# world-modelz/world-modelz

Hardware: AMD Instinct MI355X
Metric: denoise-step latent-frames/sec (forward, 32x16x16 latent clips) (higher is better)
Workload: dtype bf16; 1 GPU; BASELINE.json configs[3] per GPU: VqVideoDiffusionModel.forward, B=8 clips/GPU of 32x16x16 latents, codebook 1024, dim 256, dim_head 128, heads 1, extents 3,3,3, depth 4, mlp 256; clips_per_gpu=8, codebook=1024, parallelism=clips sharded over 1 rank(s), no data-path collective

## Files before the change

### world_modelz_amd/csrc/fused_common.h

```cpp
#pragma once
#include "wmz_common.h"
#include <stdlib.h>

#define WMZ_FENCE()                        \
  do {                                     \
    asm volatile("" ::: "memory");         \
    __builtin_amdgcn_sched_barrier(0);     \
  } while (0)

namespace {

constexpr int TW = 32;
#ifndef WMZ_FUSED_FW
#define WMZ_FUSED_FW 8
#endif
constexpr int FW = WMZ_FUSED_FW;
constexpr int NTHR = FW * 64;
constexpr int HALF = 16384;
constexpr int PIECES = HALF / 1024;
#ifndef WMZ_FUSED_HPS
#define WMZ_FUSED_HPS 2
#endif
constexpr int HPS = WMZ_FUSED_HPS;
constexpr int SLAB = HPS * HALF;
#ifndef WMZ_FUSED_RING
#define WMZ_FUSED_RING (WMZ_FUSED_HPS == 1 ? 4 : 2)
#endif
constexpr int RING = WMZ_FUSED_RING;
constexpr int WPP = SLAB / 1024 / FW;
constexpr int VECB = 8192;
constexpr int MC = 32;

struct WStream {
  int dbg;
  const char* src;
  char* ring;
  int issue_slot;
  int cur;
  int half;
  int wave;
  int probe;
  long long* ts;
  int tot, t1, t2, t3;
  int all;
};

__device__ __forceinline__ void ws_issue(WStream& ws) {
  ws.t1 = ws.t2; ws.t2 = ws.t3; ws.t3 = ws.tot;
  ws.all += WPP;
  if (ws.dbg & 2) return;
  char* dst = ws.ring + ws.issue_slot * SLAB;
#pragma unroll
  for (int i = 0; i < WPP; ++i)
    __builtin_amdgcn_global_load_lds((const __attribute__((address_space(1))) void*)(ws.src + i * 1024),
                                     (__attribute__((address_space(3))) void*)(dst + i * 1024), 16, 0, 0);
  ws.src += SLAB;
  ws.issue_slot = ws.issue_slot == RING - 1 ? 0 : ws.issue_slot + 1;
}

__device__ __forceinline__ void ws_wait(WStream& ws) {
  constexpr int YB = WPP * (RING - 2);
  static_assert(YB == 4 || YB == 0, "literals below");
  const int e = ws.tot - (RING == 4 ? ws.t1 : (RING == 3 ? ws.t2 : ws.t3));
  if (!(ws.dbg & 2)) {
#define WMZ_VMC(n) case n: if (YB == 4) asm volatile("s_waitcnt vmcnt(" #n " + 4)" ::: "memory"); else asm volatile("s_waitcnt vmcnt(" #n ")" ::: "memory"); break;
    switch (e) {
      WMZ_VMC(0) WMZ_VMC(1) WMZ_VMC(2) WMZ_VMC(3) WMZ_VMC(4) WMZ_VMC(5) WMZ_VMC(6) WMZ_VMC(7) WMZ_VMC(8) WMZ_VMC(9)
      WMZ_VMC(10) WMZ_VMC(11) WMZ_VMC(12) WMZ_VMC(13) WMZ_VMC(14) WMZ_VMC(15) WMZ_VMC(16) WMZ_VMC(17) WMZ_VMC(18)
      WMZ_VMC(19) WMZ_VMC(20) WMZ_VMC(21) WMZ_VMC(22) WMZ_VMC(23) WMZ_VMC(24) WMZ_VMC(25) WMZ_VMC(26) WMZ_VMC(27)
      WMZ_VMC(28) WMZ_VMC(29) WMZ_VMC(30) WMZ_VMC(31) WMZ_VMC(32)
      default: asm volatile("s_waitcnt vmcnt(32)" ::: "memory"); break;
    }
#undef WMZ_VMC
  }
  if (ws.probe && ws.ts) ws.ts[ws.probe] = __builtin_readcyclecounter();
  if (!(ws.dbg & 4)) __builtin_amdgcn_s_barrier();
  if (ws.probe && ws.ts) ws.ts[ws.probe + 1] = __builtin_readcyclecounter();
}
__device__ __forceinline__ void ws_release(WStream& ws) { ws.cur = ws.cur == RING - 1 ? 0 : ws.cur + 1; }
__device__ __forceinline__ void ws_extra(WStream& ws, int n) { ws.tot += n; ws.all += n; }
__device__ __forceinline__ void vm_wait(int n) {
#define WMZ_VMW(k) case k: asm volatile("s_waitcnt vmcnt(" #k ")" ::: "memory"); break;
  switch (n) {
    WMZ_VMW(0) WMZ_VMW(1) WMZ_VMW(2) WMZ_VMW(3) WMZ_VMW(4) WMZ_VMW(5) WMZ_VMW(6) WMZ_VMW(7) WMZ_VMW(8) WMZ_VMW(9) WMZ_VMW(10)
    WMZ_VMW(11) WMZ_VMW(12) WMZ_VMW(13) WMZ_VMW(14) WMZ_VMW(15) WMZ_VMW(16) WMZ_VMW(17) WMZ_VMW(18) WMZ_VMW(19) WMZ_VMW(20)
    WMZ_VMW(21) WMZ_VMW(22) WMZ_VMW(23) WMZ_VMW(24) WMZ_VMW(25) WMZ_VMW(26) WMZ_VMW(27) WMZ_VMW(28) WMZ_VMW(29) WMZ_VMW(30)
    WMZ_VMW(31) WMZ_VMW(32) WMZ_VMW(33) WMZ_VMW(34) WMZ_VMW(35) WMZ_VMW(36) WMZ_VMW(37) WMZ_VMW(38) WMZ_VMW(39) WMZ_VMW(40)
    WMZ_VMW(41) WMZ_VMW(42) WMZ_VMW(43) WMZ_VMW(44) WMZ_VMW(45) WMZ_VMW(46) WMZ_VMW(47)
    default: asm volatile("s_waitcnt vmcnt(48)" ::: "memory"); break;
  }
#undef WMZ_VMW
}
__device__ __forceinline__ void vm_wait_since(const WStream& ws, int mark) { vm_wait(ws.all - mark); }

struct NoSide { static constexpr int kValuPerMfma = 0; __device__ __forceinline__ void operator()(int) const {} };
template <int VPM, typename F> struct SideWork {
  static constexpr int kValuPerMfma = VPM;
  F f;
  __device__ __forceinline__ void operator()(int g) const { f(g); }
};
template <int VPM, typename F> __device__ __forceinline__ SideWork<VPM, F> side_work(F f) { return SideWork<VPM, F>{f}; }

template <int NB, int KS, typename BGet, typename Side = NoSide>
__device__ __forceinline__ void gemm_stage_b(f32x16 (&acc)[NB], BGet bget, const char* ring0, WStream& ws, int lane,
                                             Side side = Side()) {
  constexpr int NP = NB * KS;
  static_assert(NP % PIECES == 0, "a stage is a whole number of slabs");
  constexpr int AG = 4, GPS = PIECES / AG;
  Frag8<bf16_t> bcur, bnext = bget(0);
  bcur = bnext;
#pragma unroll
  for (int sl = 0; sl < NP / PIECES; ++sl) {
    if (ws.half == 0) ws_wait(ws);
    const char* slab = ring0 + ws.cur * SLAB + ws.half * HALF + lane * 16;
    Frag8<bf16_t> af[2][AG];
    if (!(ws.dbg & 1)) {
#pragma unroll
      for (int j = 0; j < AG; ++j) af[0][j].v = *reinterpret_cast<const s16x8*>(slab + j * 1024);
    }
    if (ws.half == 0) ws_issue(ws);
    if (ws.probe && ws.ts) ws.ts[ws.probe + 2] = __builtin_readcyclecounter();
    if (!(ws.dbg & 1)) {
#pragma unroll
      for (int gq = 0; gq < GPS; ++gq) {
        if (gq == 1 && ws.probe && ws.ts) { asm volatile("s_waitcnt lgkmcnt(0)" ::: "memory"); ws.ts[ws.probe + 3] = __builtin_readcyclecounter(); }
        if (gq + 1 < GPS) {
#pragma unroll
          for (int j = 0; j < AG; ++j)
            af[(gq + 1) & 1][j].v = *reinterpret_cast<const s16x8*>(slab + ((gq + 1) * AG + j) * 1024);
        }
#pragma unroll
        for (int j = 0; j < AG; ++j) {
          const int idx = sl * PIECES + gq * AG + j;
          if (idx % NB == 0) {
            bcur = bnext;
            if (idx / NB + 1 < KS) bnext = bget(idx / NB + 1);
          }
          mma32(acc[idx % NB], af[gq & 1][j], bcur);
        }
        side(sl * GPS + gq);
        if (gq + 1 < GPS) __builtin_amdgcn_sched_group_barrier(0x100, AG, 0);
        if constexpr (Side::kValuPerMfma > 0) {
#pragma unroll
          for (int j = 0; j < AG; ++j) {
            __builtin_amdgcn_sched_group_barrier(0x008, 1, 0);
            __builtin_amdgcn_sched_group_barrier(0x002, Side::kValuPerMfma, 0);
          }
        } else {
          __builtin_amdgcn_sched_group_barrier(0x008, AG, 0);
        }
        WMZ_FENCE();
      }
    }
    if (ws.half == HPS - 1) { ws_release(ws); ws.half = 0; }
    else ++ws.half;
  }
}
template <int NB, int KS, typename Side = NoSide>
__device__ __forceinline__ void gemm_stage(f32x16 (&acc)[NB], const Frag8<bf16_t> (&bop)[KS], const char* ring0, WStream& ws,
                                           int lane, Side side = Side()) {
  gemm_stage_b<NB, KS>(acc, [&](int s) { return bop[s]; }, ring0, ws, lane, side);
}

__device__ __forceinline__ f32x16 lds_vec16(const float* p) {
  const f32x4 a = *reinterpret_cast<const f32x4*>(p), b = *reinterpret_cast<const f32x4*>(p + 4);
  const f32x4 c = *reinterpret_cast<const f32x4*>(p + 8), d = *reinterpret_cast<const f32x4*>(p + 12);
  f32x16 v;
#pragma unroll
  for (int i = 0; i < 4; ++i) { v[i] = a[i]; v[4 + i] = b[i]; v[8 + i] = c[i]; v[12 + i] = d[i]; }
  return v;
}
template <int NB>
__device__ __forceinline__ void add_vec(f32x16 (&acc)[NB], const float* vec ) {
#pragma unroll
  for (int b = 0; b < NB; ++b) acc[b] += lds_vec16(vec + 16 * b);
}
template <int NB>
__device__ __forceinline__ void init_vec(f32x16 (&acc)[NB], const float* vec) {
#pragma unroll
  for (int b = 0; b < NB; ++b) acc[b] = lds_vec16(vec + 16 * b);
}

__device__ __forceinline__ void pack8(Frag8<bf16_t>& f, const float (&y)[8]) {
#ifdef WMZ_OP16_F16
  const s16x4 lo = cvt_pk4_bf16(y[0], y[1], y[2], y[3]), hi = cvt_pk4_bf16(y[4], y[5], y[6], y[7]);
  s16x8 v = __builtin_shufflevector(lo, hi, 0, 1, 2, 3, 4, 5, 6, 7);
#else
  s16x8 v;
#pragma unroll
  for (int j = 0; j < 8; ++j) v[j] = (short)f32_to_bf16_bits(y[j]);
#endif
  asm volatile("" : "+v"(v));
  f.v = v;
}

template <int KS>
__device__ __forceinline__ void load_bop(Frag8<bf16_t> (&bop)[KS], const bf16_t* half_row) {
#pragma unroll
  for (int s = 0; s < KS; ++s) bop[s].v = *reinterpret_cast<const s16x8*>(half_row + 8 * s);
}

__device__ __forceinline__ s16x8 gload_untracked(const bf16_t* p) {
  s16x8 v;
  asm volatile("global_load_dwordx4 %0, %1, off" : "=v"(v) : "v"(p) : "memory");
  return v;
}
template <int KS>
__device__ __forceinline__ void wait_untracked(Frag8<bf16_t> (&b)[KS]) {
  if (WPP * (RING - 1) == 6) asm volatile("s_waitcnt vmcnt(6)" ::: "memory");
  else asm volatile("s_waitcnt vmcnt(4)" ::: "memory");
#pragma unroll
  for (int s = 0; s < KS; ++s) asm volatile("" : "+v"(b[s].v));
}
__device__ __forceinline__ void vec_dma(float* vecs, const float* src, int wave, int lane) {
#pragma unroll
  for (int i = 0; i < 8 / FW; ++i) {
    const int kb = wave * (8 / FW) + i;
    __builtin_amdgcn_global_load_lds((const __attribute__((address_space(1))) void*)(src + kb * 256 + lane * 4),
                                     (__attribute__((address_space(3))) void*)(reinterpret_cast<char*>(vecs) + kb * 1024), 16, 0, 0);
  }
}
template <int NB>
__device__ __forceinline__ void add_bop(f32x16 (&acc)[NB], const Frag8<bf16_t> (&bop)[2 * NB]) {
#pragma unroll
  for (int b = 0; b < NB; ++b)
#pragma unroll
    for (int i = 0; i < 16; ++i) acc[b][i] = op16_add_to(acc[b][i], (unsigned short)bop[2 * b + (i >> 3)].v[i & 7]);
}

template <int KS>
__device__ __forceinline__ void load_bop_tiled(Frag8<bf16_t> (&bop)[KS], const bf16_t* tile, int lane) {
#pragma unroll
  for (int s = 0; s < KS; ++s) bop[s].v = *reinterpret_cast<const s16x8*>(tile + (s * 64 + lane) * 8);
}
template <int KS>
__device__ __forceinline__ void store_bop_tiled(bf16_t* tile, const Frag8<bf16_t> (&bop)[KS], int lane, HalfGuard& hg) {
  if (hg.on()) {
#pragma unroll
    for (int s = 0; s < KS; ++s) hg.see(bop[s].v);
    hg.fold(WMZ_HG_STREAM);
  }
#pragma unroll
  for (int s = 0; s < KS; ++s) *reinterpret_cast<s16x8*>(tile + (s * 64 + lane) * 8) = bop[s].v;
}

__device__ __forceinline__ void stage_dma128(char* stg, const bf16_t* src, int rowf, long tok0, int ntok, int lane) {
#pragma unroll
  for (int p = 0; p < 8; ++p) {
    const int r = p * 4 + (lane >> 4), pc = lane & 15;
    const long row = tok0 + r < ntok ? tok0 + r : ntok - 1;
    __builtin_amdgcn_global_load_lds((const __attribute__((address_space(1))) void*)(src + row * rowf + ((pc ^ (r & 15)) << 3)),
                                     (__attribute__((address_space(3))) void*)(stg + p * 1024), 16, 0, 0);
  }
}
__device__ __forceinline__ Frag8<bf16_t> stage_get(const char* stg, int t, int c) {
  Frag8<bf16_t> f;
  f.v = *reinterpret_cast<const s16x8*>(stg + t * 256 + ((c ^ (t & 15)) << 4));
  return f;
}
__device__ __forceinline__ void stage_put(char* stg, const s16x8& v, int t, int c) {
  *reinterpret_cast<s16x8*>(stg + t * 256 + ((c ^ (t & 15)) << 4)) = v;
}
template <int ROWF>
__device__ __forceinline__ void stage_flush(const char* stg, bf16_t* dst, long tok0, int ntok, int col0, int lane, HalfGuard& hg,
                                            unsigned kind) {
  asm volatile("" : "+s"(tok0), "+v"(lane));
  s16x8 v[8];
#pragma unroll
  for (int p = 0; p < 8; ++p) v[p] = *reinterpret_cast<const s16x8*>(stg + p * 1024 + lane * 16);
  if (hg.on()) {
#pragma unroll
    for (int p = 0; p < 8; ++p) hg.see(v[p]);
    hg.fold(kind);
  }
#pragma unroll
  for (int p = 0; p < 8; ++p) {
    const int r = p * 4 + (lane >> 4), pc = lane & 15;
    const int c = pc ^ (r & 15);
    if (tok0 + r < ntok) *reinterpret_cast<s16x8*>(dst + (tok0 + r) * ROWF + col0 + c * 8) = v[p];
  }
}
template <int ROWF>
__device__ __forceinline__ void stage_flush(const char* stg, bf16_t* dst, long tok0, int ntok, int col0, int lane) {
  HalfGuard none;
  stage_flush<ROWF>(stg, dst, tok0, ntok, col0, lane, none, 0u);
}
__device__ __forceinline__ void frag_park(char* stg, int slot, const Frag8<bf16_t>& f, int lane) {
  *reinterpret_cast<s16x8*>(stg + slot * 1024 + lane * 16) = f.v;
}
__device__ __forceinline__ Frag8<bf16_t> frag_unpark(const char* stg, int slot, int lane) {
  Frag8<bf16_t> f;
  f.v = *reinterpret_cast<const s16x8*>(stg + slot * 1024 + lane * 16);
  return f;
}

__device__ __forceinline__ void store_tile128(char* stg, bf16_t* dst, int rowf, long tok0, int ntok, int col0,
                                              const Frag8<bf16_t> (&b)[8], int lane, HalfGuard& hg) {
  const int t = lane & 31, h = lane >> 5;
#pragma unroll
  for (int s = 0; s < 8; ++s) stage_put(stg, b[s].v, t, h * 8 + s);
  if (rowf == 128) stage_flush<128>(stg, dst, tok0, ntok, col0, lane, hg, WMZ_HG_QKV);
  else stage_flush<256>(stg, dst, tok0, ntok, col0, lane, hg, WMZ_HG_QKV);
}
__device__ __forceinline__ void store_tile128(char* stg, bf16_t* dst, int rowf, long tok0, int ntok, int col0,
                                              const Frag8<bf16_t> (&b)[8], int lane) {
  HalfGuard none;
  store_tile128(stg, dst, rowf, tok0, ntok, col0, b, lane, none);
}
__device__ __forceinline__ void store_tile256(char* stg, bf16_t* dst, long tok0, int ntok, const Frag8<bf16_t> (&b)[16],
                                              int lane, HalfGuard& hg) {
  const int t = lane & 31, h = lane >> 5;
#pragma unroll
  for (int hh = 0; hh < 2; ++hh) {
    if (h == hh) {
#pragma unroll
      for (int s = 0; s < 16; ++s) stage_put(stg, b[s].v, t, s);
    }
    stage_flush<256>(stg, dst, tok0, ntok, hh * 128, lane, hg, WMZ_HG_STREAM);
  }
}
__device__ __forceinline__ void store_tile256(char* stg, bf16_t* dst, long tok0, int ntok, const Frag8<bf16_t> (&b)[16],
                                              int lane) {
  HalfGuard none;
  store_tile256(stg, dst, tok0, ntok, b, lane, none);
}

template <int NB>
__device__ __forceinline__ void acc_from_bop(f32x16 (&acc)[NB], const Frag8<bf16_t> (&bop)[2 * NB]) {
#pragma unroll
  for (int b = 0; b < NB; ++b)
#pragma unroll
    for (int i = 0; i < 16; ++i) acc[b][i] = bf16_bits_to_f32((unsigned short)bop[2 * b + (i >> 3)].v[i & 7]);
#ifdef WMZ_OP16_F16
#pragma unroll
  for (int b = 0; b < NB; ++b) asm volatile("" : "+v"(acc[b]));
#endif
}
template <int NB>
__device__ __forceinline__ void bop_from_acc(Frag8<bf16_t> (&bop)[2 * NB], const f32x16 (&acc)[NB]) {
#pragma unroll
  for (int b = 0; b < NB; ++b)
#pragma unroll
    for (int m = 0; m < 2; ++m) {
      float y[8];
#pragma unroll
      for (int j = 0; j < 8; ++j) y[j] = acc[b][8 * m + j];
      pack8(bop[2 * b + m], y);
    }
}

template <int NB>
__device__ __forceinline__ void ln_stats(const f32x16 (&acc)[NB], float eps, float& rstd, float& mr) {
  constexpr int NF = NB * 32;
  f32x16 sv = acc[0];
#pragma unroll
  for (int b = 1; b < NB; ++b) sv += acc[b];
  float s = 0.f;
#pragma unroll
  for (int i = 0; i < 16; ++i) s += sv[i];
  s = wave_halves_sum(s);
  const float mean = s / (float)NF;
  f32x16 qv = (f32x16)(0.f);
#pragma unroll
  for (int b = 0; b < NB; ++b) { const f32x16 d = acc[b] - mean; qv += d * d; }
  float q = 0.f;
#pragma unroll
  for (int i = 0; i < 16; ++i) q += qv[i];
  q = wave_halves_sum(q);
  rstd = rsqrtf(q / (float)NF + eps);
  mr = -mean * rstd;
}
__device__ __forceinline__ void ln_block(Frag8<bf16_t>& lo, Frag8<bf16_t>& hi, const f32x16& x, float rstd, float mr) {
  const f32x16 y = x * rstd + mr;
  float a[8], b[8];
#pragma unroll
  for (int j = 0; j < 8; ++j) { a[j] = y[j]; b[j] = y[8 + j]; }
  pack8(lo, a);
  pack8(hi, b);
}
__device__ __forceinline__ void put_stats(float* st, long tok, int ntok, float rstd, float mr, int lane) {
  if (lane < 32 && tok < ntok) {
    st[tok] = -mr / rstd;
    st[(long)ntok + tok] = rstd;
  }
}
template <int NB>
__device__ __forceinline__ void ln_to_bop(Frag8<bf16_t> (&bop)[2 * NB], const f32x16 (&acc)[NB], float eps, float* st = nullptr,
                                          long tok = 0, int ntok = 0, int lane = 0) {
  float rstd, mr;
  ln_stats<NB>(acc, eps, rstd, mr);
  if (st != nullptr) put_stats(st, tok, ntok, rstd, mr, lane);
#pragma unroll
  for (int b = 0; b < NB; ++b) ln_block(bop[2 * b], bop[2 * b + 1], acc[b], rstd, mr);
}
template <int NB>
__device__ __forceinline__ void ln_and_pack(Frag8<bf16_t> (&lnb)[2 * NB], Frag8<bf16_t> (&xb)[2 * NB], const f32x16 (&acc)[NB],
                                            float eps, float* st = nullptr, long tok = 0, int ntok = 0, int lane = 0) {
  float rstd, mr;
  ln_stats<NB>(acc, eps, rstd, mr);
  if (st != nullptr) put_stats(st, tok, ntok, rstd, mr, lane);
#pragma unroll
  for (int b = 0; b < NB; ++b) {
    ln_block(lnb[2 * b], lnb[2 * b + 1], acc[b], rstd, mr);
    float a[8], c[8];
#pragma unroll
    for (int j = 0; j < 8; ++j) { a[j] = acc[b][j]; c[j] = acc[b][8 + j]; }
    pack8(xb[2 * b], a);
    pack8(xb[2 * b + 1], c);
  }
}

template <int N> __device__ __forceinline__ void zero_acc(f32x16 (&acc)[N]) {
#pragma unroll
  for (int b = 0; b < N; ++b) acc[b] = (f32x16)(0.f);
}
}
```

### world_modelz_amd/csrc/layer_fused.hip

```cpp
#include "fused_common.h"
#include "fused_pack_rows.h"
#include "wmz_debug.h"

namespace {

struct FusedParams {
  const bf16_t* o;
  const bf16_t* x;
  bf16_t* xo;
  bf16_t* q;
  bf16_t* kv;
  const char* wpack;
  const float* vec;
  int ntok;
  float eps;
  const int64_t* z; const float *emb, *pos_s, *pos_h, *pos_w; int S, H, W, num_classes;
  int dbg;
  int rows_out, rows_in, row0;
  int xflags;
  bf16_t* x1o; bf16_t* xo_rm; int kv_combined;
  float* st_ff; float* st_attn;
  bf16_t* zt;
  long long* ts;
};
#define WMZ_TS(slot)                                                                                      \
  do {                                                                                                    \
    if (P.ts != nullptr && blockIdx.x == 0 && lane == 0) P.ts[wave * 64 + (slot)] = __builtin_readcyclecounter(); \
  } while (0)
__device__ __forceinline__ long src_row(const FusedParams& P, long t) {
  if (P.rows_out == 0) return t;
  const int c = (int)t / P.rows_out;
  return (long)c * P.rows_in + P.row0 + ((int)t - c * P.rows_out);
}

template <int F>
__device__ __forceinline__ void embed_bop(Frag8<bf16_t> (&bop)[F / 16], const FusedParams& P, long t, bool ok, int h) {
  (void)ok;
  const long ts = src_row(P, t);
  const int w = (int)(ts % P.W), hh = (int)((ts / P.W) % P.H), s = (int)((ts / ((long)P.W * P.H)) % P.S);
  long tk = P.z[ts];
  tk = tk < 0 ? 0 : (tk >= P.num_classes ? P.num_classes - 1 : tk);
  const float* e = P.emb + tk * F + h * (F / 2);
  const float* a = P.pos_s + (long)s * F + h * (F / 2);
  const float* b = P.pos_h + (long)hh * F + h * (F / 2);
  const float* d = P.pos_w + (long)w * F + h * (F / 2);
#pragma unroll
  for (int c = 0; c < F / 16; ++c) {
    float y[8];
#pragma unroll
    for (int q = 0; q < 2; ++q) {
      const f32x4 ev = *reinterpret_cast<const f32x4*>(e + 8 * c + 4 * q);
      const f32x4 av = *reinterpret_cast<const f32x4*>(a + 8 * c + 4 * q);
      const f32x4 bv = *reinterpret_cast<const f32x4*>(b + 8 * c + 4 * q);
      const f32x4 dv = *reinterpret_cast<const f32x4*>(d + 8 * c + 4 * q);
      const f32x4 yv = ev + ((av + bv) + dv);
#pragma unroll
      for (int r = 0; r < 4; ++r) y[4 * q + r] = yv[r];
    }
    pack8(bop[c], y);
    if ((c & 1) == 1) WMZ_FENCE();
  }
}

template <int F>
__device__ __forceinline__ void embed_coop(Frag8<bf16_t> (&bop)[F / 16], char* stg, const FusedParams& P, long tok0, int lane) {
  static_assert(F == 256, "one 1 KB fp32 row per wave instruction");
  const long last = P.ntok - 1;
  const long ts0 = src_row(P, tok0 < last ? tok0 : last);
  const int h0 = (int)((ts0 / 16) % P.H), s = (int)((ts0 / (16L * P.H)) % P.S);
  const int h1 = h0 + 1 < P.H ? h0 + 1 : h0;
  const f32x4 ps = *reinterpret_cast<const f32x4*>(P.pos_s + (long)s * F + lane * 4);
  const f32x4 a0 = ps + *reinterpret_cast<const f32x4*>(P.pos_h + (long)h0 * F + lane * 4);
  const f32x4 a1 = ps + *reinterpret_cast<const f32x4*>(P.pos_h + (long)h1 * F + lane * 4);
  f32x4 pw[16];
#pragma unroll
  for (int w = 0; w < 16; ++w) pw[w] = *reinterpret_cast<const f32x4*>(P.pos_w + (long)w * F + lane * 4);
  const int t = lane & 31, hl = lane >> 5;
  int tkv;
  {
    const long tt = tok0 + t < last ? tok0 + t : last;
    long tk = P.z[ts0 + (tt - (tok0 < last ? tok0 : last))];
    tk = tk < 0 ? 0 : (tk >= P.num_classes ? P.num_classes - 1 : tk);
    tkv = (int)tk;
  }
#pragma unroll
  for (int p = 0; p < 2; ++p) {
    const f32x4 a = p ? a1 : a0;
#pragma unroll
    for (int i = 0; i < 16; ++i) {
      const long tk = __builtin_amdgcn_readlane(tkv, 16 * p + i);
      const f32x4 e = *reinterpret_cast<const f32x4*>(P.emb + tk * F + lane * 4);
      const f32x4 y = e + (a + pw[i]);
      s16x4 pk;
#pragma unroll
      for (int r = 0; r < 4; ++r) pk[r] = (short)f32_to_bf16_bits(y[r]);
      *reinterpret_cast<s16x4*>(stg + i * 512 + ((((lane >> 1) ^ i) << 4) | ((lane & 1) << 3))) = pk;
    }
    if ((t >> 4) == p) {
      const int tl = t & 15;
#pragma unroll
      for (int c = 0; c < F / 16; ++c)
        bop[c].v = *reinterpret_cast<const s16x8*>(stg + tl * 512 + (((hl * 16 + c) ^ tl) << 4));
    }
  }
}

__device__ __forceinline__ void store_z_tiled(bf16_t* zt, long tok0, int c, const f32x16& z, int lane) {
#pragma unroll
  for (int j = 0; j < 2; ++j) {
    float y[8];
#pragma unroll
    for (int i = 0; i < 8; ++i) y[i] = z[8 * j + i];
    Frag8<bf16_t> f;
    pack8(f, y);
    *reinterpret_cast<s16x8*>(zt + tok0 * 256 + ((2 * c + j) * 64 + lane) * 8) = f.v;
  }
}

template <int D, int I, int M, bool HEAD, bool TAIL>
__global__ __launch_bounds__(NTHR, 8 / FW) void layer_fused_kernel(FusedParams P) {
  static_assert(D == 256 && M == 256 && I == 128, "built for the default denoiser widths");
  extern __shared__ __attribute__((aligned(16))) char smem[];
  const int tid = threadIdx.x, lane = tid & 63;
  const int wave = __builtin_amdgcn_readfirstlane(tid >> 6);
  const int h = lane >> 5;
  float* vecs = reinterpret_cast<float*>(smem);
  const char* ring0 = smem + VECB;
  HalfGuard hg;
  WStream ws;
  ws.ring = smem + VECB + wave * (SLAB / FW);
  ws.src = P.wpack + wave * (SLAB / FW) + lane * 16;
  ws.half = 0;
  ws.issue_slot = 0;
  ws.cur = 0;
  ws.dbg = P.dbg;
  ws.tot = ws.t1 = ws.t2 = ws.t3 = 0;
  ws.all = 0;
  ws.wave = wave;
  ws.probe = 0;
  ws.ts = (P.ts != nullptr && blockIdx.x == 0 && lane == 0) ? P.ts + wave * 64 : nullptr;
  WMZ_TS(0);
  const long tok0 = (long)blockIdx.x * (TW * FW) + wave * TW;
  const long tok = tok0 + (lane & 31);
  const long tokc = tok < P.ntok ? tok : P.ntok - 1;
  const bool tile_ok = tok0 < P.ntok;
  const long tok0c = tile_ok ? tok0 : (P.ntok >= 32 ? P.ntok - 32 : 0);
  char* stg = smem + VECB + RING * SLAB + wave * 8192;
  static_assert(VECB == 8192 && 8 % FW == 0, "vector block is 2048 floats, 8 / FW KB per wave");
  const float* v_bout = vecs + h * (D / 2);
  const float* v_b1 = vecs + D + h * (MC / 2);
  const float* v_b2 = vecs + D + M + h * (D / 2);
  const float* v_bk = vecs + 2 * D + M + h * (I / 2);
  const float* v_bv = v_bk + I;

  Frag8<bf16_t> qkvb[I / 16];
  f32x16 xr[D / 32];
  Frag8<bf16_t> xb[D / 16];
  if constexpr (HEAD) {
    stage_dma128(stg, P.o, I, tok0, P.ntok, lane);
    vec_dma(vecs, P.vec, wave, lane);
#pragma unroll
    for (int i = 0; i < RING - 1; ++i) ws_issue(ws);
    const bool xt = (P.xflags & WMZ_FUSED_X_IN_TILED) != 0;
    {
      const bf16_t* xp = xt ? P.x + src_row(P, tok0c) * D + lane * 8 : P.x + src_row(P, tokc) * D + h * (D / 2);
      const int xs = xt ? 64 * 8 : 8;
#pragma unroll
      for (int s = 0; s < D / 16; ++s) xb[s].v = gload_untracked(xp + s * xs);
    }
    ws_extra(ws, D / 16);
    WMZ_TS(1);
    if (WPP * (RING - 1) == 6) asm volatile("s_waitcnt vmcnt(22)" ::: "memory");
    else asm volatile("s_waitcnt vmcnt(20)" ::: "memory");
    static_assert(WPP * (RING - 1) == 6 || WPP * (RING - 1) == 4, "literals above");
    __builtin_amdgcn_s_barrier();
    WMZ_TS(44);
    init_vec<D / 32>(xr, v_bout);
    WMZ_TS(2);
    {
      const int t = lane & 31;
      gemm_stage_b<D / 32, I / 16>(xr, [&](int ks) { return stage_get(stg, t, h * (I / 16) + ks); }, ring0, ws, lane);
    }
    wait_untracked<D / 16>(xb);
    WMZ_TS(45);
    add_bop<D / 32>(xr, xb);
    const bool x1_hat = (P.xflags & WMZ_FUSED_X1_NORMALISED) != 0;
    if (P.x1o != nullptr && !x1_hat) {
      bop_from_acc<D / 32>(xb, xr);
      store_tile256(stg, P.x1o, tok0, P.ntok, xb, lane, hg);
      ws_extra(ws, 16);
    }
    WMZ_TS(3);
    ln_to_bop<D / 32>(xb, xr, P.eps, P.st_ff, tok, P.ntok, lane);
    if (P.st_ff != nullptr) ws_extra(ws, 2);
    if (P.x1o != nullptr && x1_hat) {
      store_tile256(stg, P.x1o, tok0, P.ntok, xb, lane, hg);
      ws_extra(ws, 16);
    }
    WMZ_TS(4);
#pragma unroll
    for (int sx = 8; sx < 16; ++sx) frag_park(stg, sx - 8, xb[sx], lane);
    {
      auto lnb = [&](int sx) { return sx < 8 ? xb[sx] : frag_unpark(stg, sx - 8, lane); };
      auto gelu_n = [&](float (&y)[8], const f32x16& zz, int first, int yo, int n) {
#pragma unroll
        for (int j = 0; j < 4; ++j) if (j < n) y[yo + j] = wmz_gelu_fast(zz[first + j]);
      };
      f32x16 zc[1], zn[1];
      Frag8<bf16_t> gb[2], gn[2];
      float y[8];
      init_vec<1>(zc, v_b1);
      gemm_stage_b<1, D / 16>(zc, lnb, ring0, ws, lane);
      const bool zsave = P.zt != nullptr && tile_ok;
      if (zsave) { store_z_tiled(P.zt, tok0, 0, zc[0], lane); ws_extra(ws, 2); }
      WMZ_TS(5);
      init_vec<1>(zn, v_b1 + MC);
      gemm_stage_b<1, D / 16>(zn, lnb, ring0, ws, lane, side_work<9>([&](int g) {
        gelu_n(y, zc[0], 4 * g, (g & 1) * 4, 4);
        if (g & 1) pack8(gb[g >> 1], y);
      }));
      if (zsave) { store_z_tiled(P.zt, tok0, 1, zn[0], lane); ws_extra(ws, 2); }
      zc[0] = zn[0];
      WMZ_TS(6);
#pragma unroll 1
      for (int c = 1; c < M / MC - 1; ++c) {
        if (c == 4) ws.probe = 48;
        gemm_stage<D / 32, MC / 16>(xr, gb, ring0, ws, lane, side_work<5>([&](int g) {
          gelu_n(y, zc[0], 2 * g, 2 * g, 2);
          if (g == 3) pack8(gn[0], y);
        }));
        ws.probe = 0;
        WMZ_TS(5 + 3 * c);
        init_vec<1>(zn, v_b1 + (c + 1) * MC);
        if (c == 4) ws.probe = 52;
        gemm_stage_b<1, D / 16>(zn, lnb, ring0, ws, lane, side_work<5>([&](int g) {
          gelu_n(y, zc[0], 8 + 2 * g, 2 * g, 2);
          if (g == 3) pack8(gn[1], y);
        }));
        ws.probe = 0;
        if (zsave) { store_z_tiled(P.zt, tok0, c + 1, zn[0], lane); ws_extra(ws, 2); }
        WMZ_TS(7 + 3 * c);
        zc[0] = zn[0];
        gb[0] = gn[0];
        gb[1] = gn[1];
      }
      gemm_stage<D / 32, MC / 16>(xr, gb, ring0, ws, lane, side_work<9>([&](int g) {
        gelu_n(y, zc[0], 4 * g, (g & 1) * 4, 4);
        if (g & 1) pack8(gn[g >> 1], y);
      }));
      gemm_stage<D / 32, MC / 16>(xr, gn, ring0, ws, lane);
      WMZ_TS(29);
    }
    add_vec<D / 32>(xr, v_b2);
    Frag8<bf16_t> x2b[D / 16];
    if constexpr (TAIL) {
      ln_and_pack<D / 32>(xb, x2b, xr, P.eps, P.st_attn, tok, P.ntok, lane);
      if (P.st_attn != nullptr) ws_extra(ws, 2);
    }
    else bop_from_acc<D / 32>(x2b, xr);
    WMZ_TS(30);
    if (P.xflags & WMZ_FUSED_X_OUT_TILED) { if (tile_ok) store_bop_tiled<D / 16>(P.xo + tok0 * D, x2b, lane, hg); }
    else store_tile256(stg, P.xo, tok0, P.ntok, x2b, lane, hg);
    ws_extra(ws, 16);
    if (P.xo_rm != nullptr) {
      if (TAIL && (P.xflags & WMZ_FUSED_XRM_NORMALISED)) store_tile256(stg, P.xo_rm, tok0, P.ntok, xb, lane, hg);
      else store_tile256(stg, P.xo_rm, tok0, P.ntok, x2b, lane, hg);
      ws_extra(ws, 16);
    }
    WMZ_TS(31);
    if constexpr (TAIL) {
      f32x16 qa[I / 32];
      zero_acc(qa);
      gemm_stage<I / 32, D / 16>(qa, x2b, ring0, ws, lane);
      WMZ_TS(32);
      bop_from_acc<I / 32>(qkvb, qa);
    }
  } else {
    if (P.z != nullptr) {
      const bool coop = P.W == 16 && (P.H * 16) % 32 == 0 && (P.rows_out == 0 || (P.rows_out % 32 == 0 && P.rows_in % 32 == 0 && P.row0 % 32 == 0));
      if (coop) embed_coop<D>(xb, stg, P, tok0, lane);
      else embed_bop<D>(xb, P, tokc, true, h);
    }
    else if (P.xflags & WMZ_FUSED_X_IN_TILED) load_bop_tiled<D / 16>(xb, P.x + src_row(P, tok0c) * D, lane);
    else load_bop<D / 16>(xb, P.x + src_row(P, tokc) * D + h * (D / 2));
    f32x4 vecv[8 / FW];
#pragma unroll
    for (int i = 0; i < 8 / FW; ++i) vecv[i] = *reinterpret_cast<const f32x4*>(P.vec + (tid + i * NTHR) * 4);
#pragma unroll
    for (int i = 0; i < RING - 1; ++i) ws_issue(ws);
#pragma unroll
    for (int i = 0; i < 8 / FW; ++i) *reinterpret_cast<f32x4*>(vecs + (tid + i * NTHR) * 4) = vecv[i];
    __syncthreads();
    if (P.z != nullptr) {
      if (P.xflags & WMZ_FUSED_X_OUT_TILED) { if (tile_ok) store_bop_tiled<D / 16>(P.xo + tok0 * D, xb, lane, hg); }
      else store_tile256(stg, P.xo, tok0, P.ntok, xb, lane, hg);
      ws_extra(ws, 16);
      if (P.xo_rm != nullptr && !(P.xflags & WMZ_FUSED_XRM_NORMALISED)) { store_tile256(stg, P.xo_rm, tok0, P.ntok, xb, lane, hg); ws_extra(ws, 16); }
    }
    {
      f32x16 qa[I / 32];
      zero_acc(qa);
      gemm_stage<I / 32, D / 16>(qa, xb, ring0, ws, lane);
      bop_from_acc<I / 32>(qkvb, qa);
    }
    acc_from_bop<D / 32>(xr, xb);
    ln_to_bop<D / 32>(xb, xr, P.eps, P.st_attn, tok, P.ntok, lane);
    if (P.st_attn != nullptr) ws_extra(ws, 2);
    if (P.xo_rm != nullptr && (P.xflags & WMZ_FUSED_XRM_NORMALISED)) { store_tile256(stg, P.xo_rm, tok0, P.ntok, xb, lane, hg); ws_extra(ws, 16); }
  }
  if constexpr (TAIL) {
    f32x16 ka[I / 32];
    Frag8<bf16_t> kb[I / 16];
    init_vec<I / 32>(ka, v_bk);
    store_tile128(stg, P.q, I, tok0, P.ntok, 0, qkvb, lane, hg);
    ws_extra(ws, 8);
    WMZ_TS(33);
    gemm_stage<I / 32, D / 16>(ka, xb, ring0, ws, lane);
    WMZ_TS(34);
    bop_from_acc<I / 32>(kb, ka);
    if (P.kv_combined) store_tile128(stg, P.kv, 2 * I, tok0, P.ntok, 0, kb, lane, hg);
    else store_tile128(stg, P.kv, I, tok0, P.ntok, 0, kb, lane, hg);
    ws_extra(ws, 8);
    init_vec<I / 32>(ka, v_bv);
    WMZ_TS(35);
    gemm_stage<I / 32, D / 16>(ka, xb, ring0, ws, lane);
    WMZ_TS(36);
    bop_from_acc<I / 32>(kb, ka);
    if (P.kv_combined) store_tile128(stg, P.kv, 2 * I, tok0, P.ntok, I, kb, lane, hg);
    else store_tile128(stg, P.kv + (long)P.ntok * I, I, tok0, P.ntok, 0, kb, lane, hg);
  }
  asm volatile("s_waitcnt vmcnt(0)" ::: "memory");
  hg.commit();
  WMZ_TS(37);
}

}

static int fused_launch(FusedParams& P, int ntok, int D, int I, int M, int has_head, int has_tail, void* stream);
static FusedParams fused_params(const void* o, const void* x, void* x_out, void* q_out, void* kv_out, const void* wpack,
                                const float* vec, int ntok, float eps) {
  FusedParams P = {};
  P.o = (const bf16_t*)o; P.x = (const bf16_t*)x; P.xo = (bf16_t*)x_out; P.q = (bf16_t*)q_out; P.kv = (bf16_t*)kv_out;
  P.wpack = (const char*)wpack; P.vec = vec; P.ntok = ntok; P.eps = eps;
  return P;
}
static long long* g_fused_ts = nullptr;
static int g_fused_dbg = 0;
#ifndef WMZ_OP16_F16
extern "C" int wmz_debug_fused_knobs(int dbg) { g_fused_dbg = dbg; return WMZ_OK; }
extern "C" int wmz_debug_fused_timestamps(void* buf) { g_fused_ts = (long long*)buf; return WMZ_OK; }
#endif

extern "C" int WMZ_FN(wmz_layer_fused_fwd)(const void* o, const void* x, void* x_out, void* q_out, void* kv_out,
                                   const void* wpack, const float* vec, int ntok, int D, int I, int M, int has_head,
                                   int has_tail, float eps, void* stream) {
  return WMZ_FN(wmz_layer_fused_fwd_planes)(o, x, x_out, q_out, kv_out, wpack, vec, 1, 1, 1, ntok, D, I, M, has_head, has_tail, 0,
                                    eps, stream);
}

namespace {
struct PackRows { FusedPackRow row[24]; int n; long total8, padded8; };
struct VecJobG { const float *bout, *b1, *w1, *be2, *b2, *wk, *wv, *be1, *bv; float* vec; };
static_assert(sizeof(VecJobG) == 80, "table layouts are part of the C ABI");

__device__ __forceinline__ void pack_group(const FusedPackRow& B, long g) {
  const long e = g * 8;
  const int NB = (int)B.N / 32;
  const int piece = (int)(e / 512), lane = (int)((e % 512) / 8);
  const int s = piece / NB, b = piece % NB;
  const int r = lane & 31, h = lane >> 5;
  const int bpg = (int)B.gn / 32, spg = (int)B.gk / 16;
  const int f = (b / bpg) * (int)B.gn + ((r >> 2) & 1) * ((int)B.gn / 2) + (b % bpg) * 16 + (r & 3) + 4 * (r >> 3);
  const int k0 = (s / spg) * (int)B.gk + h * ((int)B.gk / 2) + (s % spg) * 8;
  const float rg = B.rgamma ? B.rgamma[f] : 1.f;
  s16x8 v;
#pragma unroll
  for (int j = 0; j < 8; ++j) {
    float x = B.w[(long)f * B.rs + (long)(k0 + j) * B.ks] * rg;
    if (B.gamma) x *= B.gamma[k0 + j];
    v[j] = (short)f32_to_bf16_bits(x);
  }
  *reinterpret_cast<s16x8*>(B.dst + e) = v;
}
__global__ __launch_bounds__(256) void fused_pack_kernel(PackRows P) {
  const long g8 = (long)blockIdx.x * 256 + threadIdx.x;
  if (g8 < P.total8) {
    int bi = 0;
#pragma unroll 1
    for (int i = 1; i < P.n; ++i) if (g8 >= P.row[i].start8) bi = i;
    const FusedPackRow& B = P.row[bi];
    pack_group(B, g8 - B.start8);
  } else if (g8 < P.padded8) {
    *reinterpret_cast<s16x8*>(P.row[0].dst + g8 * 8) = (s16x8)(0);
  }
}
__global__ __launch_bounds__(256) void fused_pack_table_kernel(const FusedPackRow* __restrict__ rows, int nblk, long total8) {
  const long g8 = (long)blockIdx.x * 256 + threadIdx.x;
  if (g8 >= total8) return;
  int lo = 0, hi = nblk - 1;
  while (lo < hi) {
    const int mid = (lo + hi + 1) >> 1;
    if (rows[mid].start8 <= g8) lo = mid; else hi = mid - 1;
  }
  const FusedPackRow B = rows[lo];
  pack_group(B, g8 - B.start8);
}

__device__ __forceinline__ void pack_vec_entry(const VecJobG& P, int t, int lane, int D, int I, int M) {
  const float* row = nullptr; const float* vecb = nullptr; float base = 0.f;
  if (t < D) base = P.bout ? P.bout[t] : 0.f;
  else if (t < D + M) { if (P.b1) { base = P.b1[t - D]; row = P.w1 + (long)(t - D) * D; vecb = P.be2; } }
  else if (t < 2 * D + M) base = P.b2 ? P.b2[t - D - M] : 0.f;
  else if (t < 2 * D + M + I) { if (P.wk) { row = P.wk + (long)(t - 2 * D - M) * D; vecb = P.be1; } }
  else if (t < 2 * D + M + 2 * I) { if (P.wv) { base = P.bv[t - 2 * D - M - I]; row = P.wv + (long)(t - 2 * D - M - I) * D; vecb = P.be1; } }
  float acc = 0.f;
  if (row != nullptr) {
    const f32x4 a = *reinterpret_cast<const f32x4*>(row + lane * 4), b = *reinterpret_cast<const f32x4*>(vecb + lane * 4);
    acc = a[0] * b[0] + a[1] * b[1] + a[2] * b[2] + a[3] * b[3];
    acc = wave_sum(acc);
  }
  if (lane == 0) P.vec[t] = base + acc;
}
__global__ __launch_bounds__(256) void fused_pack_vec_kernel(VecJobG P, int D, int I, int M) {
  const int t = blockIdx.x * 4 + (threadIdx.x >> 6), lane = threadIdx.x & 63;
  if (t < 2048) pack_vec_entry(P, t, lane, D, I, M);
}
__global__ __launch_bounds__(256) void fused_pack_vec_table_kernel(const VecJobG* __restrict__ jobs, int D, int I, int M) {
  const VecJobG P = jobs[blockIdx.y];
  const int t = blockIdx.x * 4 + (threadIdx.x >> 6), lane = threadIdx.x & 63;
  if (t < 2048) pack_vec_entry(P, t, lane, D, I, M);
}

void fused_pack_launch(PackRows& P, hipStream_t stream) {
  P.total8 = fused_rows_groups(P.row, P.n);
  P.padded8 = P.total8 + 65536 / 2 / 8;
  hipLaunchKernelGGL(fused_pack_kernel, dim3((unsigned)wmz_cdiv(P.padded8, 256)), dim3(256), 0, stream, P);
}
}

extern "C" int WMZ_FN(wmz_layer_fused_pack)(const float* wout, const float* bout, const float* g2, const float* be2, const float* w1,
                                    const float* b1, const float* w2, const float* b2, const float* g1, const float* be1,
                                    const float* wq, const float* wk, const float* wv, const float* bv, void* wpack,
                                    float* vec, int D, int I, int M, void* stream) {
  const bool head = wout != nullptr, tail = wq != nullptr;
  WMZ_REQUIRE(wpack && vec && (head || tail), "wmz_layer_fused_pack: bad arguments");
  WMZ_REQUIRE(D == 256 && I == 128 && M == 256, "wmz_layer_fused_pack: built for dim 256 / inner 128 / mlp 256");
  WMZ_REQUIRE(!head || (bout && g2 && be2 && w1 && b1 && w2 && b2), "wmz_layer_fused_pack: head parameters missing");
  WMZ_REQUIRE(!tail || (g1 && be1 && wk && wv && bv), "wmz_layer_fused_pack: tail parameters missing");
  const float* const p[14] = {wout, bout, g2, be2, w1, b1, w2, b2, g1, be1, wq, wk, wv, bv};
  PackRows P;
  P.n = fused_fwd_rows(P.row, p, (unsigned short*)wpack, 0);
  fused_pack_launch(P, (hipStream_t)stream);
  const VecJobG J{head ? bout : nullptr, head ? b1 : nullptr, w1, be2, head ? b2 : nullptr,
                  tail ? wk : nullptr, tail ? wv : nullptr, be1, bv, vec};
  hipLaunchKernelGGL(fused_pack_vec_kernel, dim3(512), dim3(256), 0, (hipStream_t)stream, J, D, I, M);
  WMZ_LAUNCH_CHECK("wmz_layer_fused_pack");
  return WMZ_OK;
}

extern "C" int WMZ_FN(wmz_fused_pack_table)(const void* block_rows, int nblk, long total8, const void* vec_jobs, int nvec, int D, int I,
                                    int M, void* stream) {
  WMZ_REQUIRE(nblk >= 0 && nvec >= 0 && (nblk == 0 || (block_rows && total8 > 0)) && (nvec == 0 || vec_jobs),
              "wmz_fused_pack_table: bad arguments");
  WMZ_REQUIRE(D == 256 && I == 128 && M == 256, "wmz_fused_pack_table: built for dim 256 / inner 128 / mlp 256");
  if (nblk > 0)
    hipLaunchKernelGGL(fused_pack_table_kernel, dim3((unsigned)wmz_cdiv(total8, 256)), dim3(256), 0, (hipStream_t)stream,
                       (const FusedPackRow*)block_rows, nblk, total8);
  if (nvec > 0)
    hipLaunchKernelGGL(fused_pack_vec_table_kernel, dim3(512, (unsigned)nvec), dim3(256), 0, (hipStream_t)stream,
                       (const VecJobG*)vec_jobs, D, I, M);
  WMZ_LAUNCH_CHECK("wmz_fused_pack_table");
  return WMZ_OK;
}

#ifndef WMZ_OP16_F16
extern "C" int wmz_layer_fused_bwd_pack(const float* wq, const float* wk, const float* wv, const float* g1, const float* wout,
                                        const float* w1, const float* g2, const float* w2, void* wpack_qkv, void* wpack_ff,
                                        int D, int I, int M, void* stream) {
  WMZ_REQUIRE(D == 256 && I == 128 && M == 256, "wmz_layer_fused_bwd_pack: built for dim 256 / inner 128 / mlp 256");
  WMZ_REQUIRE(wpack_qkv || wpack_ff, "wmz_layer_fused_bwd_pack: nothing to do");
  WMZ_REQUIRE(!wpack_qkv || (wq && wk && wv && g1), "wmz_layer_fused_bwd_pack: attention parameters missing");
  WMZ_REQUIRE(!wpack_ff || (wout && w1 && g2 && w2), "wmz_layer_fused_bwd_pack: feed-forward parameters missing");
  const float* const p[8] = {wq, wk, wv, g1, wout, w1, g2, w2};
  PackRows P;
  if (wpack_qkv) { P.n = fused_bwd_qkv_rows(P.row, p, (unsigned short*)wpack_qkv, 0); fused_pack_launch(P, (hipStream_t)stream); }
  if (wpack_ff) { P.n = fused_bwd_ff_rows(P.row, p, (unsigned short*)wpack_ff, 0); fused_pack_launch(P, (hipStream_t)stream); }
  WMZ_LAUNCH_CHECK("wmz_layer_fused_bwd_pack");
  return WMZ_OK;
}

extern "C" int wmz_fused_pack_rows(int kind, const void* const* params, void* dst, long start8, int D, int I, int M, void* rows_out) {
  const float* const* p = (const float* const*)params;
  FusedPackRow* rows = (FusedPackRow*)rows_out;
  const bool have = !p ? false
      : kind == FUSED_STREAM_FWD ? (p[0] || p[10]) && (!p[0] || (p[2] && p[4] && p[6])) && (!p[10] || (p[8] && p[11] && p[12]))
      : kind == FUSED_STREAM_BWD_QKV ? p[0] && p[1] && p[2] && p[3] : kind == FUSED_STREAM_BWD_FF && p[4] && p[5] && p[6] && p[7];
  const char* bad = !(have && dst && rows && start8 >= 0) ? "wmz_fused_pack_rows: bad arguments"
      : !(D == 256 && I == 128 && M == 256) ? "wmz_fused_pack_rows: built for dim 256 / inner 128 / mlp 256" : nullptr;
  if (bad != nullptr) { wmz_set_error("%s", bad); return -WMZ_ERR_ARG; }
  return kind == FUSED_STREAM_FWD ? fused_fwd_rows(rows, p, (unsigned short*)dst, start8)
       : kind == FUSED_STREAM_BWD_QKV ? fused_bwd_qkv_rows(rows, p, (unsigned short*)dst, start8)
                                      : fused_bwd_ff_rows(rows, p, (unsigned short*)dst, start8);
}

extern "C" int wmz_layer_fused_fwd_train(const void* o, const void* x, void* x_out, void* x_out_rowmajor, void* x1_out,
                                         void* q_out, void* kv_out, float* ln_ff_stats, float* ln_attn_stats,
                                         void* z_tiled_out, const void* wpack, const float* vec, int ntok, int D, int I,
                                         int M, int has_head, int has_tail, int xflags, float eps, void* stream) {
  WMZ_REQUIRE(x && wpack && vec && ntok > 0, "wmz_layer_fused_fwd_train: bad arguments");
  WMZ_REQUIRE(has_head || has_tail, "wmz_layer_fused_fwd_train: nothing to do");
  WMZ_REQUIRE(!has_head || (o && x_out), "wmz_layer_fused_fwd_train: head needs o and x_out");
  WMZ_REQUIRE(!has_tail || (q_out && kv_out), "wmz_layer_fused_fwd_train: tail needs q_out and kv_out");
  WMZ_REQUIRE((xflags & ~15) == 0 && ((xflags & 3) == 0 || ntok % 32 == 0), "wmz_layer_fused_fwd_train: bad layout flags");
  WMZ_REQUIRE(!(xflags & WMZ_FUSED_XRM_NORMALISED) || (has_tail && x_out_rowmajor && (xflags & WMZ_FUSED_X_OUT_TILED)),
              "wmz_layer_fused_fwd_train: WMZ_FUSED_XRM_NORMALISED needs the tail, x_rm_out and a tiled x_out (the raw stream must survive somewhere)");
  WMZ_REQUIRE(!(xflags & WMZ_FUSED_X1_NORMALISED) || (has_head && x1_out), "wmz_layer_fused_fwd_train: WMZ_FUSED_X1_NORMALISED needs the head and x1_out");
  FusedParams P = fused_params(o, x, x_out, q_out, kv_out, wpack, vec, ntok, eps);
  P.xflags = xflags;
  P.x1o = (bf16_t*)x1_out; P.xo_rm = (bf16_t*)x_out_rowmajor; P.kv_combined = 1;
  P.st_ff = ln_ff_stats; P.st_attn = has_tail ? ln_attn_stats : nullptr;
  WMZ_REQUIRE(z_tiled_out == nullptr || (has_head && ntok % 32 == 0), "wmz_layer_fused_fwd_train: z_tiled_out needs the head and whole 32-token tiles");
  P.zt = (bf16_t*)z_tiled_out;
  return fused_launch(P, ntok, D, I, M, has_head, has_tail, stream);
}

extern "C" int wmz_embed_qkv_fused_fwd_train(const int64_t* z, const float* emb, const float* pos_s, const float* pos_h,
                                             const float* pos_w, void* x_out, void* x_out_rowmajor, void* q_out,
                                             void* kv_out, float* ln_attn_stats, const void* wpack, const float* vec, int B,
                                             int S, int H, int W, int D, int I, int M, int num_classes, int xflags, float eps,
                                             void* stream) {
  WMZ_REQUIRE(z && emb && pos_s && pos_h && pos_w && x_out && q_out && kv_out && wpack && vec, "wmz_embed_qkv_fused_fwd_train: null tensor");
  WMZ_REQUIRE(B > 0 && S > 0 && H > 0 && W > 0 && num_classes > 0 && (long)B * S * H * W < (1L << 31), "wmz_embed_qkv_fused_fwd_train: bad shape");
  WMZ_REQUIRE((xflags & ~(WMZ_FUSED_X_OUT_TILED | WMZ_FUSED_XRM_NORMALISED)) == 0 && (xflags == 0 || ((long)S * H * W) % 32 == 0), "wmz_embed_qkv_fused_fwd_train: bad layout flags");
  WMZ_REQUIRE(!(xflags & WMZ_FUSED_XRM_NORMALISED) || (x_out_rowmajor && (xflags & WMZ_FUSED_X_OUT_TILED)),
              "wmz_embed_qkv_fused_fwd_train: WMZ_FUSED_XRM_NORMALISED needs x_out_rowmajor and a tiled x_out");
  FusedParams P = fused_params(nullptr, nullptr, x_out, q_out, kv_out, wpack, vec, B * S * H * W, eps);
  P.z = z; P.emb = emb; P.pos_s = pos_s; P.pos_h = pos_h; P.pos_w = pos_w; P.S = S; P.H = H; P.W = W; P.num_classes = num_classes;
  P.xflags = xflags;
  P.xo_rm = (bf16_t*)x_out_rowmajor; P.kv_combined = 1;
  P.st_attn = ln_attn_stats;
  return fused_launch(P, P.ntok, D, I, M, 0, 1, stream);
}

#endif

extern "C" int WMZ_FN(wmz_layer_fused_fwd_planes)(const void* o, const void* x, void* x_out, void* q_out, void* kv_out,
                                          const void* wpack, const float* vec, int B, int planes_out, int planes_in, int HW,
                                          int D, int I, int M, int has_head, int has_tail, int xflags, float eps,
                                          void* stream) {
  WMZ_REQUIRE((xflags & ~3) == 0, "wmz_layer_fused_fwd: bad layout flags");
  WMZ_REQUIRE(xflags == 0 || ((long)planes_out * HW) % 32 == 0 && ((long)planes_in * HW) % 32 == 0,
              "wmz_layer_fused_fwd: the tiled stream layout needs whole 32-token tiles per clip");
  WMZ_REQUIRE(B > 0 && HW > 0 && planes_out > 0 && planes_out <= planes_in, "wmz_layer_fused_fwd: bad plane counts");
  WMZ_REQUIRE((long)B * planes_in * HW < (1L << 31), "wmz_layer_fused_fwd: token count overflows int");
  const int ntok = B * planes_out * HW;
  WMZ_REQUIRE(x && wpack && vec && ntok > 0, "wmz_layer_fused_fwd: bad arguments");
  WMZ_REQUIRE(has_head || has_tail, "wmz_layer_fused_fwd: nothing to do");
  WMZ_REQUIRE(!has_head || (o && x_out), "wmz_layer_fused_fwd: head needs o and x_out");
  WMZ_REQUIRE(!has_tail || (q_out && kv_out), "wmz_layer_fused_fwd: tail needs q_out and kv_out");
  FusedParams P = fused_params(o, x, x_out, q_out, kv_out, wpack, vec, ntok, eps);
  if (planes_out != planes_in) { P.rows_out = planes_out * HW; P.rows_in = planes_in * HW; P.row0 = (planes_in - planes_out) * HW; }
  P.xflags = xflags;
  return fused_launch(P, ntok, D, I, M, has_head, has_tail, stream);
}

extern "C" int WMZ_FN(wmz_embed_qkv_fused_fwd)(const int64_t* z, const float* emb, const float* pos_s, const float* pos_h,
                                       const float* pos_w, void* x_out, void* q_out, void* kv_out, const void* wpack,
                                       const float* vec, int B, int S, int H, int W, int D, int I, int M, int num_classes,
                                       float eps, void* stream) {
  return WMZ_FN(wmz_embed_qkv_fused_fwd_planes)(z, emb, pos_s, pos_h, pos_w, x_out, q_out, kv_out, wpack, vec, B, S, H, W, S, D, I, M,
                                        num_classes, 0, eps, stream);
}

extern "C" int WMZ_FN(wmz_embed_qkv_fused_fwd_planes)(const int64_t* z, const float* emb, const float* pos_s, const float* pos_h,
                                              const float* pos_w, void* x_out, void* q_out, void* kv_out, const void* wpack,
                                              const float* vec, int B, int S, int H, int W, int planes_out, int D, int I,
                                              int M, int num_classes, int xflags, float eps, void* stream) {
  WMZ_REQUIRE((xflags & ~WMZ_FUSED_X_OUT_TILED) == 0, "wmz_embed_qkv_fused_fwd: bad layout flags");
  WMZ_REQUIRE(xflags == 0 || ((long)planes_out * H * W) % 32 == 0, "wmz_embed_qkv_fused_fwd: the tiled stream layout needs whole 32-token tiles per clip");
  WMZ_REQUIRE(planes_out > 0 && planes_out <= S, "wmz_embed_qkv_fused_fwd: bad plane count");
  WMZ_REQUIRE((long)B * S * H * W < (1L << 31), "wmz_embed_qkv_fused_fwd: token count overflows int");
  WMZ_REQUIRE(z && emb && pos_s && pos_h && pos_w && x_out && q_out && kv_out && wpack && vec, "wmz_embed_qkv_fused_fwd: null tensor");
  WMZ_REQUIRE(B > 0 && S > 0 && H > 0 && W > 0 && num_classes > 0, "wmz_embed_qkv_fused_fwd: bad shape");
  FusedParams P = fused_params(nullptr, nullptr, x_out, q_out, kv_out, wpack, vec, B * planes_out * H * W, eps);
  if (planes_out != S) { P.rows_out = planes_out * H * W; P.rows_in = S * H * W; P.row0 = (S - planes_out) * H * W; }
  P.z = z; P.emb = emb; P.pos_s = pos_s; P.pos_h = pos_h; P.pos_w = pos_w; P.S = S; P.H = H; P.W = W; P.num_classes = num_classes;
  P.xflags = xflags;
  return fused_launch(P, P.ntok, D, I, M, 0, 1, stream);
}

static int fused_launch(FusedParams& P, int ntok, int D, int I, int M, int has_head, int has_tail, void* stream) {
  if (!(D == 256 && I == 128 && M == 256)) {
    wmz_set_error("wmz_layer_fused_fwd: built for dim 256 / inner 128 / mlp 256 (got %d/%d/%d); use the unfused path", D, I, M);
    return WMZ_ERR_UNSUPPORTED;
  }
  P.dbg = g_fused_dbg;
  P.ts = g_fused_ts;
  const size_t smem = VECB + RING * SLAB + FW * 8192;
  dim3 grid((unsigned)wmz_cdiv(ntok, TW * FW)), block(NTHR);
  hipStream_t st = (hipStream_t)stream;
#define WMZ_FUSED(H, T)                                                                                            \
  do {                                                                                                             \
    auto kern = layer_fused_kernel<256, 128, 256, H, T>;                                                           \
    (void)hipFuncSetAttribute(reinterpret_cast<const void*>(kern), hipFuncAttributeMaxDynamicSharedMemorySize, 160 * 1024); \
    hipLaunchKernelGGL(kern, grid, block, smem, st, P);                                                            \
  } while (0)
  if (has_head && has_tail) WMZ_FUSED(true, true);
  else if (has_head) WMZ_FUSED(true, false);
  else WMZ_FUSED(false, true);
#undef WMZ_FUSED
  WMZ_LAUNCH_CHECK("wmz_layer_fused_fwd");
  return WMZ_OK;
}
```

Baseline: 742,400 latent-frames/s.

## Specialize fused layer kernel for plain layout without debug and timestamp paths

Templates the fused layer kernel on PLAIN and TS flags, so the common case (whole tiles, no remapped rows, no side outputs, no debug knobs) compiles without bounds clamps, row remapping, debug branches and timestamp probes. In that path the x-input load is deferred (X_LATE) and uses SGPR-based untracked loads, and whole-tile staging DMA and stores drop the per-row bounds checks. The aim is less scalar/vector overhead and register pressure, plus looser vmcnt waits. In exchange it adds more kernel instantiations and host-side dispatch logic, and the late x load changes the wait accounting in a way that could stall.

```diff
diff --git a/world_modelz_amd/csrc/fused_common.h b/world_modelz_amd/csrc/fused_common.h
--- a/world_modelz_amd/csrc/fused_common.h
+++ b/world_modelz_amd/csrc/fused_common.h
@@ -31,7 +31,9 @@
 constexpr int VECB = 8192;
 constexpr int MC = 32;
 
-struct WStream {
+template <bool PLAIN_, bool TS_>
+struct WStreamT {
+  static constexpr bool PLAIN = PLAIN_, TS = TS_;
   int dbg;
   const char* src;
   char* ring;
@@ -44,11 +46,13 @@
   int tot, t1, t2, t3;
   int all;
 };
-
-__device__ __forceinline__ void ws_issue(WStream& ws) {
+typedef WStreamT<false, false> WStream;
+
+template <typename WS>
+__device__ __forceinline__ void ws_issue(WS& ws) {
   ws.t1 = ws.t2; ws.t2 = ws.t3; ws.t3 = ws.tot;
   ws.all += WPP;
-  if (ws.dbg & 2) return;
+  if constexpr (!WS::PLAIN) { if (ws.dbg & 2) return; }
   char* dst = ws.ring + ws.issue_slot * SLAB;
 #pragma unroll
   for (int i = 0; i < WPP; ++i)
@@ -58,11 +62,12 @@
   ws.issue_slot = ws.issue_slot == RING - 1 ? 0 : ws.issue_slot + 1;
 }
 
-__device__ __forceinline__ void ws_wait(WStream& ws) {
+template <typename WS>
+__device__ __forceinline__ void ws_wait(WS& ws) {
   constexpr int YB = WPP * (RING - 2);
   static_assert(YB == 4 || YB == 0, "literals below");
   const int e = ws.tot - (RING == 4 ? ws.t1 : (RING == 3 ? ws.t2 : ws.t3));
-  if (!(ws.dbg & 2)) {
+  if (WS::PLAIN || !(ws.dbg & 2)) {
 #define WMZ_VMC(n) case n: if (YB == 4) asm volatile("s_waitcnt vmcnt(" #n " + 4)" ::: "memory"); else asm volatile("s_waitcnt vmcnt(" #n ")" ::: "memory"); break;
     switch (e) {
       WMZ_VMC(0) WMZ_VMC(1) WMZ_VMC(2) WMZ_VMC(3) WMZ_VMC(4) WMZ_VMC(5) WMZ_VMC(6) WMZ_VMC(7) WMZ_VMC(8) WMZ_VMC(9)
@@ -73,12 +78,12 @@
     }
 #undef WMZ_VMC
   }
-  if (ws.probe && ws.ts) ws.ts[ws.probe] = __builtin_readcyclecounter();
-  if (!(ws.dbg & 4)) __builtin_amdgcn_s_barrier();
-  if (ws.probe && ws.ts) ws.ts[ws.probe + 1] = __builtin_readcyclecounter();
-}
-__device__ __forceinline__ void ws_release(WStream& ws) { ws.cur = ws.cur == RING - 1 ? 0 : ws.cur + 1; }
-__device__ __forceinline__ void ws_extra(WStream& ws, int n) { ws.tot += n; ws.all += n; }
+  if constexpr (WS::TS) { if (ws.probe && ws.ts) ws.ts[ws.probe] = __builtin_readcyclecounter(); }
+  if (WS::PLAIN || !(ws.dbg & 4)) __builtin_amdgcn_s_barrier();
+  if constexpr (WS::TS) { if (ws.probe && ws.ts) ws.ts[ws.probe + 1] = __builtin_readcyclecounter(); }
+}
+template <typename WS> __device__ __forceinline__ void ws_release(WS& ws) { ws.cur = ws.cur == RING - 1 ? 0 : ws.cur + 1; }
+template <typename WS> __device__ __forceinline__ void ws_extra(WS& ws, int n) { ws.tot += n; ws.all += n; }
 __device__ __forceinline__ void vm_wait(int n) {
 #define WMZ_VMW(k) case k: asm volatile("s_waitcnt vmcnt(" #k ")" ::: "memory"); break;
   switch (n) {
@@ -91,7 +96,7 @@
   }
 #undef WMZ_VMW
 }
-__device__ __forceinline__ void vm_wait_since(const WStream& ws, int mark) { vm_wait(ws.all - mark); }
+template <typename WS> __device__ __forceinline__ void vm_wait_since(const WS& ws, int mark) { vm_wait(ws.all - mark); }
 
 struct NoSide { static constexpr int kValuPerMfma = 0; __device__ __forceinline__ void operator()(int) const {} };
 template <int VPM, typename F> struct SideWork {
@@ -101,9 +106,10 @@
 };
 template <int VPM, typename F> __device__ __forceinline__ SideWork<VPM, F> side_work(F f) { return SideWork<VPM, F>{f}; }
 
-template <int NB, int KS, typename BGet, typename Side = NoSide>
-__device__ __forceinline__ void gemm_stage_b(f32x16 (&acc)[NB], BGet bget, const char* ring0, WStream& ws, int lane,
+template <int NB, int KS, typename BGet, typename Side = NoSide, typename WS>
+__device__ __forceinline__ void gemm_stage_b(f32x16 (&acc)[NB], BGet bget, const char* ring0, WS& ws, int lane,
                                              Side side = Side()) {
+  constexpr bool MMA_ALWAYS = WS::PLAIN;
   constexpr int NP = NB * KS;
   static_assert(NP % PIECES == 0, "a stage is a whole number of slabs");
   constexpr int AG = 4, GPS = PIECES / AG;
@@ -114,16 +120,16 @@
     if (ws.half == 0) ws_wait(ws);
     const char* slab = ring0 + ws.cur * SLAB + ws.half * HALF + lane * 16;
     Frag8<bf16_t> af[2][AG];
-    if (!(ws.dbg & 1)) {
+    if (MMA_ALWAYS || !(ws.dbg & 1)) {
 #pragma unroll
       for (int j = 0; j < AG; ++j) af[0][j].v = *reinterpret_cast<const s16x8*>(slab + j * 1024);
     }
     if (ws.half == 0) ws_issue(ws);
-    if (ws.probe && ws.ts) ws.ts[ws.probe + 2] = __builtin_readcyclecounter();
-    if (!(ws.dbg & 1)) {
+    if constexpr (WS::TS) { if (ws.probe && ws.ts) ws.ts[ws.probe + 2] = __builtin_readcyclecounter(); }
+    if (MMA_ALWAYS || !(ws.dbg & 1)) {
 #pragma unroll
       for (int gq = 0; gq < GPS; ++gq) {
-        if (gq == 1 && ws.probe && ws.ts) { asm volatile("s_waitcnt lgkmcnt(0)" ::: "memory"); ws.ts[ws.probe + 3] = __builtin_readcyclecounter(); }
+        if constexpr (WS::TS) if (gq == 1 && ws.probe && ws.ts) { asm volatile("s_waitcnt lgkmcnt(0)" ::: "memory"); ws.ts[ws.probe + 3] = __builtin_readcyclecounter(); }
         if (gq + 1 < GPS) {
 #pragma unroll
           for (int j = 0; j < AG; ++j)
@@ -156,8 +162,8 @@
     else ++ws.half;
   }
 }
-template <int NB, int KS, typename Side = NoSide>
-__device__ __forceinline__ void gemm_stage(f32x16 (&acc)[NB], const Frag8<bf16_t> (&bop)[KS], const char* ring0, WStream& ws,
+template <int NB, int KS, typename Side = NoSide, typename WS>
+__device__ __forceinline__ void gemm_stage(f32x16 (&acc)[NB], const Frag8<bf16_t> (&bop)[KS], const char* ring0, WS& ws,
                                            int lane, Side side = Side()) {
   gemm_stage_b<NB, KS>(acc, [&](int s) { return bop[s]; }, ring0, ws, lane, side);
 }
@@ -205,6 +211,11 @@
   asm volatile("global_load_dwordx4 %0, %1, off" : "=v"(v) : "v"(p) : "memory");
   return v;
 }
+__device__ __forceinline__ s16x8 gload_untracked(const char* base, unsigned voff) {
+  s16x8 v;
+  asm volatile("global_load_dwordx4 %0, %1, %2" : "=v"(v) : "v"(voff), "s"(base) : "memory");
+  return v;
+}
 template <int KS>
 __device__ __forceinline__ void wait_untracked(Frag8<bf16_t> (&b)[KS]) {
   if (WPP * (RING - 1) == 6) asm volatile("s_waitcnt vmcnt(6)" ::: "memory");
@@ -244,7 +255,18 @@
   for (int s = 0; s < KS; ++s) *reinterpret_cast<s16x8*>(tile + (s * 64 + lane) * 8) = bop[s].v;
 }
 
+template <bool WHOLE = false>
 __device__ __forceinline__ void stage_dma128(char* stg, const bf16_t* src, int rowf, long tok0, int ntok, int lane) {
+  if constexpr (WHOLE) {
+    const char* base = reinterpret_cast<const char*>(src + tok0 * rowf);
+    const unsigned r0 = (unsigned)lane >> 4, pc = (unsigned)lane & 15u;
+    const unsigned off0 = r0 * (unsigned)(rowf * 2) + ((pc ^ r0) << 4);
+#pragma unroll
+    for (int p = 0; p < 8; ++p)
+      __builtin_amdgcn_global_load_lds((const __attribute__((address_space(1))) void*)(base + (long)(p * 4 * rowf * 2) + (off0 ^ ((p & 3u) << 6))),
+                                       (__attribute__((address_space(3))) void*)(stg + p * 1024), 16, 0, 0);
+    return;
+  }
 #pragma unroll
   for (int p = 0; p < 8; ++p) {
     const int r = p * 4 + (lane >> 4), pc = lane & 15;
@@ -261,7 +283,7 @@
 __device__ __forceinline__ void stage_put(char* stg, const s16x8& v, int t, int c) {
   *reinterpret_cast<s16x8*>(stg + t * 256 + ((c ^ (t & 15)) << 4)) = v;
 }
-template <int ROWF>
+template <int ROWF, bool WHOLE = false>
 __device__ __forceinline__ void stage_flush(const char* stg, bf16_t* dst, long tok0, int ntok, int col0, int lane, HalfGuard& hg,
                                             unsigned kind) {
   asm volatile("" : "+s"(tok0), "+v"(lane));
@@ -273,6 +295,14 @@
     for (int p = 0; p < 8; ++p) hg.see(v[p]);
     hg.fold(kind);
   }
+  if constexpr (WHOLE) {
+    char* base = reinterpret_cast<char*>(dst + tok0 * ROWF + col0);
+    const unsigned r0 = (unsigned)lane >> 4, pc = (unsigned)lane & 15u;
+    const unsigned off0 = r0 * (ROWF * 2u) + ((pc ^ r0) << 4);
+#pragma unroll
+    for (int p = 0; p < 8; ++p) *reinterpret_cast<s16x8*>(base + p * (4L * ROWF * 2) + (off0 ^ ((p & 3u) << 6))) = v[p];
+    return;
+  }
 #pragma unroll
   for (int p = 0; p < 8; ++p) {
     const int r = p * 4 + (lane >> 4), pc = lane & 15;
@@ -294,19 +324,21 @@
   return f;
 }
 
+template <bool WHOLE = false>
 __device__ __forceinline__ void store_tile128(char* stg, bf16_t* dst, int rowf, long tok0, int ntok, int col0,
                                               const Frag8<bf16_t> (&b)[8], int lane, HalfGuard& hg) {
   const int t = lane & 31, h = lane >> 5;
 #pragma unroll
   for (int s = 0; s < 8; ++s) stage_put(stg, b[s].v, t, h * 8 + s);
-  if (rowf == 128) stage_flush<128>(stg, dst, tok0, ntok, col0, lane, hg, WMZ_HG_QKV);
-  else stage_flush<256>(stg, dst, tok0, ntok, col0, lane, hg, WMZ_HG_QKV);
+  if (rowf == 128) stage_flush<128, WHOLE>(stg, dst, tok0, ntok, col0, lane, hg, WMZ_HG_QKV);
+  else stage_flush<256, WHOLE>(stg, dst, tok0, ntok, col0, lane, hg, WMZ_HG_QKV);
 }
 __device__ __forceinline__ void store_tile128(char* stg, bf16_t* dst, int rowf, long tok0, int ntok, int col0,
                                               const Frag8<bf16_t> (&b)[8], int lane) {
   HalfGuard none;
   store_tile128(stg, dst, rowf, tok0, ntok, col0, b, lane, none);
 }
+template <bool WHOLE = false>
 __device__ __forceinline__ void store_tile256(char* stg, bf16_t* dst, long tok0, int ntok, const Frag8<bf16_t> (&b)[16],
                                               int lane, HalfGuard& hg) {
   const int t = lane & 31, h = lane >> 5;
@@ -316,7 +348,7 @@
 #pragma unroll
       for (int s = 0; s < 16; ++s) stage_put(stg, b[s].v, t, s);
     }
-    stage_flush<256>(stg, dst, tok0, ntok, hh * 128, lane, hg, WMZ_HG_STREAM);
+    stage_flush<256, WHOLE>(stg, dst, tok0, ntok, hh * 128, lane, hg, WMZ_HG_STREAM);
   }
 }
 __device__ __forceinline__ void store_tile256(char* stg, bf16_t* dst, long tok0, int ntok, const Frag8<bf16_t> (&b)[16],
diff --git a/world_modelz_amd/csrc/layer_fused.hip b/world_modelz_amd/csrc/layer_fused.hip
--- a/world_modelz_amd/csrc/layer_fused.hip
+++ b/world_modelz_amd/csrc/layer_fused.hip
@@ -22,21 +22,26 @@
   float* st_ff; float* st_attn;
   bf16_t* zt;
   long long* ts;
+  int plain;
 };
 #define WMZ_TS(slot)                                                                                      \
   do {                                                                                                    \
-    if (P.ts != nullptr && blockIdx.x == 0 && lane == 0) P.ts[wave * 64 + (slot)] = __builtin_readcyclecounter(); \
+    if constexpr (TS) {                                                                                   \
+      if (P.ts != nullptr && blockIdx.x == 0 && lane == 0) P.ts[wave * 64 + (slot)] = __builtin_readcyclecounter(); \
+    }                                                                                                     \
   } while (0)
+template <bool PLAIN>
 __device__ __forceinline__ long src_row(const FusedParams& P, long t) {
+  if constexpr (PLAIN) return t;
   if (P.rows_out == 0) return t;
   const int c = (int)t / P.rows_out;
   return (long)c * P.rows_in + P.row0 + ((int)t - c * P.rows_out);
 }
 
-template <int F>
+template <int F, bool PLAIN>
 __device__ __forceinline__ void embed_bop(Frag8<bf16_t> (&bop)[F / 16], const FusedParams& P, long t, bool ok, int h) {
   (void)ok;
-  const long ts = src_row(P, t);
+  const long ts = src_row<PLAIN>(P, t);
   const int w = (int)(ts % P.W), hh = (int)((ts / P.W) % P.H), s = (int)((ts / ((long)P.W * P.H)) % P.S);
   long tk = P.z[ts];
   tk = tk < 0 ? 0 : (tk >= P.num_classes ? P.num_classes - 1 : tk);
@@ -62,12 +67,20 @@
   }
 }
 
-template <int F>
+template <int F, bool PLAIN>
 __device__ __forceinline__ void embed_coop(Frag8<bf16_t> (&bop)[F / 16], char* stg, const FusedParams& P, long tok0, int lane) {
   static_assert(F == 256, "one 1 KB fp32 row per wave instruction");
-  const long last = P.ntok - 1;
-  const long ts0 = src_row(P, tok0 < last ? tok0 : last);
-  const int h0 = (int)((ts0 / 16) % P.H), s = (int)((ts0 / (16L * P.H)) % P.S);
+  const long last = PLAIN ? 0x7fffffffL : P.ntok - 1;
+  const long ts0 = src_row<PLAIN>(P, tok0 < last ? tok0 : last);
+  int h0, s;
+  if constexpr (PLAIN) {
+    const unsigned pr = (unsigned)ts0 >> 4, ps_ = pr / (unsigned)P.H;
+    h0 = (int)(pr - ps_ * (unsigned)P.H);
+    s = (int)(ps_ % (unsigned)P.S);
+  } else {
+    h0 = (int)((ts0 / 16) % P.H);
+    s = (int)((ts0 / (16L * P.H)) % P.S);
+  }
   const int h1 = h0 + 1 < P.H ? h0 + 1 : h0;
   const f32x4 ps = *reinterpret_cast<const f32x4*>(P.pos_s + (long)s * F + lane * 4);
   const f32x4 a0 = ps + *reinterpret_cast<const f32x4*>(P.pos_h + (long)h0 * F + lane * 4);
@@ -79,7 +92,7 @@
   int tkv;
   {
     const long tt = tok0 + t < last ? tok0 + t : last;
-    long tk = P.z[ts0 + (tt - (tok0 < last ? tok0 : last))];
+    long tk = PLAIN ? P.z[tok0 + t] : P.z[ts0 + (tt - (tok0 < last ? tok0 : last))];
     tk = tk < 0 ? 0 : (tk >= P.num_classes ? P.num_classes - 1 : tk);
     tkv = (int)tk;
   }
@@ -117,33 +130,37 @@
   }
 }
 
-template <int D, int I, int M, bool HEAD, bool TAIL>
-__global__ __launch_bounds__(NTHR, 8 / FW) void layer_fused_kernel(FusedParams P) {
+template <int D, int I, int M, bool HEAD, bool TAIL, bool PLAIN, bool TS>
+__device__ __forceinline__ void layer_fused_body(const FusedParams& P) {
   static_assert(D == 256 && M == 256 && I == 128, "built for the default denoiser widths");
   extern __shared__ __attribute__((aligned(16))) char smem[];
-  const int tid = threadIdx.x, lane = tid & 63;
+  int tid = threadIdx.x;
+#ifdef WMZ_OP16_F16
+  asm volatile("" : "+v"(tid));
+#endif
+  const int lane = tid & 63;
   const int wave = __builtin_amdgcn_readfirstlane(tid >> 6);
   const int h = lane >> 5;
   float* vecs = reinterpret_cast<float*>(smem);
   const char* ring0 = smem + VECB;
   HalfGuard hg;
-  WStream ws;
+  WStreamT<PLAIN, TS> ws;
   ws.ring = smem + VECB + wave * (SLAB / FW);
   ws.src = P.wpack + wave * (SLAB / FW) + lane * 16;
   ws.half = 0;
   ws.issue_slot = 0;
   ws.cur = 0;
-  ws.dbg = P.dbg;
+  ws.dbg = PLAIN ? 0 : P.dbg;
   ws.tot = ws.t1 = ws.t2 = ws.t3 = 0;
   ws.all = 0;
   ws.wave = wave;
   ws.probe = 0;
-  ws.ts = (P.ts != nullptr && blockIdx.x == 0 && lane == 0) ? P.ts + wave * 64 : nullptr;
+  ws.ts = (TS && P.ts != nullptr && blockIdx.x == 0 && lane == 0) ? P.ts + wave * 64 : nullptr;
   WMZ_TS(0);
   const long tok0 = (long)blockIdx.x * (TW * FW) + wave * TW;
   const long tok = tok0 + (lane & 31);
-  const long tokc = tok < P.ntok ? tok : P.ntok - 1;
-  const bool tile_ok = tok0 < P.ntok;
+  const long tokc = PLAIN || tok < P.ntok ? tok : P.ntok - 1;
+  const bool tile_ok = PLAIN || tok0 < P.ntok;
   const long tok0c = tile_ok ? tok0 : (P.ntok >= 32 ? P.ntok - 32 : 0);
   char* stg = smem + VECB + RING * SLAB + wave * 8192;
   static_assert(VECB == 8192 && 8 % FW == 0, "vector block is 2048 floats, 8 / FW KB per wave");
@@ -153,24 +170,42 @@
   const float* v_bk = vecs + 2 * D + M + h * (I / 2);
   const float* v_bv = v_bk + I;
 
+#ifndef WMZ_FUSED_X_LATE
+#define WMZ_FUSED_X_LATE 1
+#endif
+  constexpr bool X_LATE = PLAIN && WMZ_FUSED_X_LATE != 0;
   Frag8<bf16_t> qkvb[I / 16];
   f32x16 xr[D / 32];
   Frag8<bf16_t> xb[D / 16];
   if constexpr (HEAD) {
-    stage_dma128(stg, P.o, I, tok0, P.ntok, lane);
+    stage_dma128<PLAIN>(stg, P.o, I, tok0, P.ntok, lane);
     vec_dma(vecs, P.vec, wave, lane);
 #pragma unroll
     for (int i = 0; i < RING - 1; ++i) ws_issue(ws);
     const bool xt = (P.xflags & WMZ_FUSED_X_IN_TILED) != 0;
-    {
-      const bf16_t* xp = xt ? P.x + src_row(P, tok0c) * D + lane * 8 : P.x + src_row(P, tokc) * D + h * (D / 2);
+    const char* xl_base = nullptr; unsigned xl_off = 0; long xl_step = 0;
+    if constexpr (PLAIN) {
+      const char* xbase = reinterpret_cast<const char*>(P.x + tok0 * D);
+      const unsigned xoff = xt ? (unsigned)lane * 16u : (unsigned)(lane & 31) * (D * 2u) + (unsigned)h * (unsigned)D;
+      const long xs = xt ? 64 * 16 : 16;
+      xl_base = xbase; xl_off = xoff; xl_step = xs;
+      if constexpr (!X_LATE) {
+#pragma unroll
+        for (int s = 0; s < D / 16; ++s) xb[s].v = gload_untracked(xbase + s * xs, xoff);
+      }
+    } else {
+      const bf16_t* xp = xt ? P.x + src_row<PLAIN>(P, tok0c) * D + lane * 8 : P.x + src_row<PLAIN>(P, tokc) * D + h * (D / 2);
       const int xs = xt ? 64 * 8 : 8;
 #pragma unroll
       for (int s = 0; s < D / 16; ++s) xb[s].v = gload_untracked(xp + s * xs);
     }
-    ws_extra(ws, D / 16);
+    if constexpr (!X_LATE) ws_extra(ws, D / 16);
     WMZ_TS(1);
-    if (WPP * (RING - 1) == 6) asm volatile("s_waitcnt vmcnt(22)" ::: "memory");
+    if constexpr (X_LATE) {
+      if (WPP * (RING - 1) == 6) asm volatile("s_waitcnt vmcnt(6)" ::: "memory");
+      else asm volatile("s_waitcnt vmcnt(4)" ::: "memory");
+    }
+    else if (WPP * (RING - 1) == 6) asm volatile("s_waitcnt vmcnt(22)" ::: "memory");
     else asm volatile("s_waitcnt vmcnt(20)" ::: "memory");
     static_assert(WPP * (RING - 1) == 6 || WPP * (RING - 1) == 4, "literals above");
     __builtin_amdgcn_s_barrier();
@@ -179,23 +214,42 @@
     WMZ_TS(2);
     {
       const int t = lane & 31;
-      gemm_stage_b<D / 32, I / 16>(xr, [&](int ks) { return stage_get(stg, t, h * (I / 16) + ks); }, ring0, ws, lane);
+      auto oget = [&](int ks) { return stage_get(stg, t, h * (I / 16) + ks); };
+      if constexpr (X_LATE) {
+        static_assert(RING == 2 && HPS == 2, "the x pieces must sit between the stage's two slab issues");
+        gemm_stage_b<D / 32, I / 16>(xr, oget, ring0, ws, lane, side_work<0>([&](int g) {
+          if (g < 4) {
+#pragma unroll
+            for (int j = 0; j < 4; ++j) xb[4 * g + j].v = gload_untracked(xl_base + (4 * g + j) * xl_step, xl_off);
+            ws_extra(ws, 4);
+          }
+        }));
+      }
+      else gemm_stage_b<D / 32, I / 16>(xr, oget, ring0, ws, lane);
     }
     wait_untracked<D / 16>(xb);
     WMZ_TS(45);
     add_bop<D / 32>(xr, xb);
     const bool x1_hat = (P.xflags & WMZ_FUSED_X1_NORMALISED) != 0;
-    if (P.x1o != nullptr && !x1_hat) {
-      bop_from_acc<D / 32>(xb, xr);
-      store_tile256(stg, P.x1o, tok0, P.ntok, xb, lane, hg);
-      ws_extra(ws, 16);
+    if constexpr (PLAIN) {
+#pragma unroll
+      for (int b = 0; b < D / 32; ++b) asm volatile("" : "+v"(xr[b]));
+    }
+    if constexpr (!PLAIN) {
+      if (P.x1o != nullptr && !x1_hat) {
+        bop_from_acc<D / 32>(xb, xr);
+        store_tile256(stg, P.x1o, tok0, P.ntok, xb, lane, hg);
+        ws_extra(ws, 16);
+      }
     }
     WMZ_TS(3);
-    ln_to_bop<D / 32>(xb, xr, P.eps, P.st_ff, tok, P.ntok, lane);
-    if (P.st_ff != nullptr) ws_extra(ws, 2);
-    if (P.x1o != nullptr && x1_hat) {
-      store_tile256(stg, P.x1o, tok0, P.ntok, xb, lane, hg);
-      ws_extra(ws, 16);
+    ln_to_bop<D / 32>(xb, xr, P.eps, PLAIN ? nullptr : P.st_ff, tok, P.ntok, lane);
+    if constexpr (!PLAIN) {
+      if (P.st_ff != nullptr) ws_extra(ws, 2);
+      if (P.x1o != nullptr && x1_hat) {
+        store_tile256(stg, P.x1o, tok0, P.ntok, xb, lane, hg);
+        ws_extra(ws, 16);
+      }
     }
     WMZ_TS(4);
 #pragma unroll
@@ -211,7 +265,7 @@
       float y[8];
       init_vec<1>(zc, v_b1);
       gemm_stage_b<1, D / 16>(zc, lnb, ring0, ws, lane);
-      const bool zsave = P.zt != nullptr && tile_ok;
+      const bool zsave = !PLAIN && P.zt != nullptr && tile_ok;
       if (zsave) { store_z_tiled(P.zt, tok0, 0, zc[0], lane); ws_extra(ws, 2); }
       WMZ_TS(5);
       init_vec<1>(zn, v_b1 + MC);
@@ -224,20 +278,20 @@
       WMZ_TS(6);
 #pragma unroll 1
       for (int c = 1; c < M / MC - 1; ++c) {
-        if (c == 4) ws.probe = 48;
+        if constexpr (TS) { if (c == 4) ws.probe = 48; }
         gemm_stage<D / 32, MC / 16>(xr, gb, ring0, ws, lane, side_work<5>([&](int g) {
           gelu_n(y, zc[0], 2 * g, 2 * g, 2);
           if (g == 3) pack8(gn[0], y);
         }));
-        ws.probe = 0;
+        if constexpr (TS) ws.probe = 0;
         WMZ_TS(5 + 3 * c);
         init_vec<1>(zn, v_b1 + (c + 1) * MC);
-        if (c == 4) ws.probe = 52;
+        if constexpr (TS) { if (c == 4) ws.probe = 52; }
         gemm_stage_b<1, D / 16>(zn, lnb, ring0, ws, lane, side_work<5>([&](int g) {
           gelu_n(y, zc[0], 8 + 2 * g, 2 * g, 2);
           if (g == 3) pack8(gn[1], y);
         }));
-        ws.probe = 0;
+        if constexpr (TS) ws.probe = 0;
         if (zsave) { store_z_tiled(P.zt, tok0, c + 1, zn[0], lane); ws_extra(ws, 2); }
         WMZ_TS(7 + 3 * c);
         zc[0] = zn[0];
@@ -254,15 +308,15 @@
     add_vec<D / 32>(xr, v_b2);
     Frag8<bf16_t> x2b[D / 16];
     if constexpr (TAIL) {
-      ln_and_pack<D / 32>(xb, x2b, xr, P.eps, P.st_attn, tok, P.ntok, lane);
-      if (P.st_attn != nullptr) ws_extra(ws, 2);
+      ln_and_pack<D / 32>(xb, x2b, xr, P.eps, PLAIN ? nullptr : P.st_attn, tok, P.ntok, lane);
+      if constexpr (!PLAIN) { if (P.st_attn != nullptr) ws_extra(ws, 2); }
     }
     else bop_from_acc<D / 32>(x2b, xr);
     WMZ_TS(30);
     if (P.xflags & WMZ_FUSED_X_OUT_TILED) { if (tile_ok) store_bop_tiled<D / 16>(P.xo + tok0 * D, x2b, lane, hg); }
-    else store_tile256(stg, P.xo, tok0, P.ntok, x2b, lane, hg);
+    else store_tile256<PLAIN>(stg, P.xo, tok0, P.ntok, x2b, lane, hg);
     ws_extra(ws, 16);
-    if (P.xo_rm != nullptr) {
+    if constexpr (!PLAIN) if (P.xo_rm != nullptr) {
       if (TAIL && (P.xflags & WMZ_FUSED_XRM_NORMALISED)) store_tile256(stg, P.xo_rm, tok0, P.ntok, xb, lane, hg);
       else store_tile256(stg, P.xo_rm, tok0, P.ntok, x2b, lane, hg);
       ws_extra(ws, 16);
@@ -277,12 +331,12 @@
     }
   } else {
     if (P.z != nullptr) {
-      const bool coop = P.W == 16 && (P.H * 16) % 32 == 0 && (P.rows_out == 0 || (P.rows_out % 32 == 0 && P.rows_in % 32 == 0 && P.row0 % 32 == 0));
-      if (coop) embed_coop<D>(xb, stg, P, tok0, lane);
-      else embed_bop<D>(xb, P, tokc, true, h);
-    }
-    else if (P.xflags & WMZ_FUSED_X_IN_TILED) load_bop_tiled<D / 16>(xb, P.x + src_row(P, tok0c) * D, lane);
-    else load_bop<D / 16>(xb, P.x + src_row(P, tokc) * D + h * (D / 2));
+      const bool coop = P.W == 16 && (P.H * 16) % 32 == 0 && (PLAIN || P.rows_out == 0 || (P.rows_out % 32 == 0 && P.rows_in % 32 == 0 && P.row0 % 32 == 0));
+      if (coop) embed_coop<D, PLAIN>(xb, stg, P, tok0, lane);
+      else embed_bop<D, PLAIN>(xb, P, tokc, true, h);
+    }
+    else if (P.xflags & WMZ_FUSED_X_IN_TILED) load_bop_tiled<D / 16>(xb, P.x + src_row<PLAIN>(P, tok0c) * D, lane);
+    else load_bop<D / 16>(xb, P.x + src_row<PLAIN>(P, tokc) * D + h * (D / 2));
     f32x4 vecv[8 / FW];
 #pragma unroll
     for (int i = 0; i < 8 / FW; ++i) vecv[i] = *reinterpret_cast<const f32x4*>(P.vec + (tid + i * NTHR) * 4);
@@ -293,9 +347,9 @@
     __syncthreads();
     if (P.z != nullptr) {
       if (P.xflags & WMZ_FUSED_X_OUT_TILED) { if (tile_ok) store_bop_tiled<D / 16>(P.xo + tok0 * D, xb, lane, hg); }
-      else store_tile256(stg, P.xo, tok0, P.ntok, xb, lane, hg);
+      else store_tile256<PLAIN>(stg, P.xo, tok0, P.ntok, xb, lane, hg);
       ws_extra(ws, 16);
-      if (P.xo_rm != nullptr && !(P.xflags & WMZ_FUSED_XRM_NORMALISED)) { store_tile256(stg, P.xo_rm, tok0, P.ntok, xb, lane, hg); ws_extra(ws, 16); }
+      if constexpr (!PLAIN) if (P.xo_rm != nullptr && !(P.xflags & WMZ_FUSED_XRM_NORMALISED)) { store_tile256(stg, P.xo_rm, tok0, P.ntok, xb, lane, hg); ws_extra(ws, 16); }
     }
     {
       f32x16 qa[I / 32];
@@ -304,35 +358,51 @@
       bop_from_acc<I / 32>(qkvb, qa);
     }
     acc_from_bop<D / 32>(xr, xb);
-    ln_to_bop<D / 32>(xb, xr, P.eps, P.st_attn, tok, P.ntok, lane);
-    if (P.st_attn != nullptr) ws_extra(ws, 2);
-    if (P.xo_rm != nullptr && (P.xflags & WMZ_FUSED_XRM_NORMALISED)) { store_tile256(stg, P.xo_rm, tok0, P.ntok, xb, lane, hg); ws_extra(ws, 16); }
+    ln_to_bop<D / 32>(xb, xr, P.eps, PLAIN ? nullptr : P.st_attn, tok, P.ntok, lane);
+    if constexpr (!PLAIN) if (P.st_attn != nullptr) ws_extra(ws, 2);
+    if constexpr (!PLAIN) if (P.xo_rm != nullptr && (P.xflags & WMZ_FUSED_XRM_NORMALISED)) { store_tile256(stg, P.xo_rm, tok0, P.ntok, xb, lane, hg); ws_extra(ws, 16); }
   }
   if constexpr (TAIL) {
     f32x16 ka[I / 32];
     Frag8<bf16_t> kb[I / 16];
     init_vec<I / 32>(ka, v_bk);
-    store_tile128(stg, P.q, I, tok0, P.ntok, 0, qkvb, lane, hg);
+    store_tile128<PLAIN>(stg, P.q, I, tok0, P.ntok, 0, qkvb, lane, hg);
     ws_extra(ws, 8);
     WMZ_TS(33);
     gemm_stage<I / 32, D / 16>(ka, xb, ring0, ws, lane);
     WMZ_TS(34);
     bop_from_acc<I / 32>(kb, ka);
-    if (P.kv_combined) store_tile128(stg, P.kv, 2 * I, tok0, P.ntok, 0, kb, lane, hg);
-    else store_tile128(stg, P.kv, I, tok0, P.ntok, 0, kb, lane, hg);
+    if (!PLAIN && P.kv_combined) store_tile128(stg, P.kv, 2 * I, tok0, P.ntok, 0, kb, lane, hg);
+    else store_tile128<PLAIN>(stg, P.kv, I, tok0, P.ntok, 0, kb, lane, hg);
     ws_extra(ws, 8);
     init_vec<I / 32>(ka, v_bv);
     WMZ_TS(35);
     gemm_stage<I / 32, D / 16>(ka, xb, ring0, ws, lane);
     WMZ_TS(36);
     bop_from_acc<I / 32>(kb, ka);
-    if (P.kv_combined) store_tile128(stg, P.kv, 2 * I, tok0, P.ntok, I, kb, lane, hg);
-    else store_tile128(stg, P.kv + (long)P.ntok * I, I, tok0, P.ntok, 0, kb, lane, hg);
+    if (!PLAIN && P.kv_combined) store_tile128(stg, P.kv, 2 * I, tok0, P.ntok, I, kb, lane, hg);
+    else store_tile128<PLAIN>(stg, P.kv + (long)P.ntok * I, I, tok0, P.ntok, 0, kb, lane, hg);
   }
   asm volatile("s_waitcnt vmcnt(0)" ::: "memory");
   hg.commit();
   WMZ_TS(37);
 }
+
+#ifndef WMZ_OP16_F16
+template <int D, int I, int M, bool HEAD, bool TAIL, bool PLAIN, bool TS>
+__global__ __launch_bounds__(NTHR, 8 / FW) void layer_fused_kernel(FusedParams P) {
+  layer_fused_body<D, I, M, HEAD, TAIL, PLAIN, TS>(P);
+}
+#else
+template <int D, int I, int M, bool HEAD, bool TAIL>
+__global__ __launch_bounds__(NTHR, 8 / FW) void layer_fused_kernel(FusedParams P) {
+  if (P.plain) {
+    layer_fused_body<D, I, M, HEAD, TAIL, true, false>(P);
+    __builtin_amdgcn_endpgm();
+  }
+  layer_fused_body<D, I, M, HEAD, TAIL, false, false>(P);
+}
+#endif
 
 }
 
@@ -344,10 +414,14 @@
   P.wpack = (const char*)wpack; P.vec = vec; P.ntok = ntok; P.eps = eps;
   return P;
 }
+#ifdef WMZ_OP16_F16
+extern int wmz_fused_dbg_knobs;
+#else
+__attribute__((visibility("hidden"))) int wmz_fused_dbg_knobs = 0;
+#endif
 static long long* g_fused_ts = nullptr;
-static int g_fused_dbg = 0;
 #ifndef WMZ_OP16_F16
-extern "C" int wmz_debug_fused_knobs(int dbg) { g_fused_dbg = dbg; return WMZ_OK; }
+extern "C" int wmz_debug_fused_knobs(int dbg) { wmz_fused_dbg_knobs = dbg; return WMZ_OK; }
 extern "C" int wmz_debug_fused_timestamps(void* buf) { g_fused_ts = (long long*)buf; return WMZ_OK; }
 #endif
 
@@ -594,20 +668,38 @@
     wmz_set_error("wmz_layer_fused_fwd: built for dim 256 / inner 128 / mlp 256 (got %d/%d/%d); use the unfused path", D, I, M);
     return WMZ_ERR_UNSUPPORTED;
   }
-  P.dbg = g_fused_dbg;
+  P.dbg = wmz_fused_dbg_knobs;
   P.ts = g_fused_ts;
   const size_t smem = VECB + RING * SLAB + FW * 8192;
   dim3 grid((unsigned)wmz_cdiv(ntok, TW * FW)), block(NTHR);
   hipStream_t st = (hipStream_t)stream;
-#define WMZ_FUSED(H, T)                                                                                            \
+  const bool plain = ntok % (TW * FW) == 0 && P.rows_out == 0 && P.x1o == nullptr && P.xo_rm == nullptr && P.st_ff == nullptr &&
+                     P.st_attn == nullptr && P.zt == nullptr && P.kv_combined == 0 && wmz_fused_dbg_knobs == 0;
+  const bool ts = g_fused_ts != nullptr;
+  P.plain = plain;
+#ifdef WMZ_OP16_F16
+#define WMZ_FUSED_KERNEL(H, T, PL, TSV) layer_fused_kernel<256, 128, 256, H, T>
+#else
+#define WMZ_FUSED_KERNEL(H, T, PL, TSV) layer_fused_kernel<256, 128, 256, H, T, PL, TSV>
+#endif
+#define WMZ_FUSED(H, T, PL, TSV)                                                                                   \
   do {                                                                                                             \
-    auto kern = layer_fused_kernel<256, 128, 256, H, T>;                                                           \
+    auto kern = WMZ_FUSED_KERNEL(H, T, PL, TSV);                                                                   \
     (void)hipFuncSetAttribute(reinterpret_cast<const void*>(kern), hipFuncAttributeMaxDynamicSharedMemorySize, 160 * 1024); \
     hipLaunchKernelGGL(kern, grid, block, smem, st, P);                                                            \
   } while (0)
-  if (has_head && has_tail) WMZ_FUSED(true, true);
-  else if (has_head) WMZ_FUSED(true, false);
-  else WMZ_FUSED(false, true);
+#define WMZ_FUSED_UNIT(H, T)                                                                                       \
+  do {                                                                                                             \
+    if (plain && ts) WMZ_FUSED(H, T, true, true);                                                                  \
+    else if (plain) WMZ_FUSED(H, T, true, false);                                                                  \
+    else if (ts) WMZ_FUSED(H, T, false, true);                                                                     \
+    else WMZ_FUSED(H, T, false, false);                                                                            \
+  } while (0)
+  if (has_head && has_tail) WMZ_FUSED_UNIT(true, true);
+  else if (has_head) WMZ_FUSED_UNIT(true, false);
+  else WMZ_FUSED_UNIT(false, true);
+#undef WMZ_FUSED_UNIT
+#undef WMZ_FUSED_KERNEL
 #undef WMZ_FUSED
   WMZ_LAUNCH_CHECK("wmz_layer_fused_fwd");
   return WMZ_OK;
```

Result: faster. 776,000 latent-frames/s (median of 6 runs) (+4.5%).
